# alibaba/TePDist

Measured on AMD Instinct MI355X. Metric: tokens/sec, higher is better.
Workload: dtype bf16; 1 GPU; model=gpt2-345m, global_batch=64, seq_len=1024, parallelism=auto-planned-graph:dp1tp1pp1mesh[]micro1

## Files before the change

### tepdist_amd/ops/build_ext.py

```python

from __future__ import annotations

import concurrent.futures as cf
import os
import subprocess
import sys
import sysconfig
from pathlib import Path

OPS_DIR = Path(__file__).resolve().parent
CSRC = OPS_DIR / "csrc"
OUT_SO = OPS_DIR / "_tepdist_hip.so"
BUILD = CSRC / "build"

HIPCC = os.environ.get("HIPCC", "/opt/rocm/bin/hipcc")
ARCH = os.environ.get("TEPDIST_GFX_ARCH", "gfx950")

SOURCES = [
    "gemm.hip",
    "gemm256.hip",
    "attention.hip",
    "decode_attention.hip",
    "transpose.hip",
    "layernorm.hip",
    "softmax.hip",
    "embedding.hip",
    "cross_entropy.hip",
    "dropout.hip",
    "elementwise.hip",
    "adamw.hip",
    "llama_ops.hip",
    "debug.hip",
    "bindings.cpp",
]


def _includes():
    import pybind11
    return [
        "-I", pybind11.get_include(),
        "-I", sysconfig.get_paths()["include"],
        "-I", str(CSRC),
    ]


def _needs_build() -> bool:
    if not OUT_SO.exists():
        return True
    so_mtime = OUT_SO.stat().st_mtime
    deps = [CSRC / s for s in SOURCES] + [CSRC / "common.h", CSRC / "kernels.h",
                                          Path(__file__)]
    return any(d.stat().st_mtime > so_mtime for d in deps)


RT_CSRC = OPS_DIR.parent / "runtime" / "csrc"
RT_SO = OPS_DIR.parent / "runtime" / "_tepdist_rt.so"
CXX = os.environ.get("CXX", "g++")


def build_rt(force: bool = False, verbose: bool = True) -> Path:
    src = RT_CSRC / "rt_core.cpp"
    if not force and RT_SO.exists() and \
            RT_SO.stat().st_mtime > src.stat().st_mtime:
        return RT_SO
    cmd = [CXX, "-O3", "-std=c++17", "-shared", "-fPIC",
           *_includes(), str(src), "-o", str(RT_SO)]
    if verbose:
        print("[build_ext]", " ".join(cmd), flush=True)
    r = subprocess.run(cmd, capture_output=True, text=True)
    if r.returncode != 0:
        raise RuntimeError(
            f"rt_core build failed:\n{r.stdout}\n{r.stderr}")
    return RT_SO


BLT_SO = OPS_DIR / "_tepdist_blt.so"


def build_blt(force: bool = False, verbose: bool = True) -> Path:
    src = CSRC / "blaslt.cpp"
    if not force and BLT_SO.exists() and \
            BLT_SO.stat().st_mtime > src.stat().st_mtime:
        return BLT_SO
    cmd = [HIPCC, "-O3", "-std=c++17", "-shared", "-fPIC",
           *_includes(), str(src), "-L", "/opt/rocm/lib", "-lhipblaslt",
           "-o", str(BLT_SO)]
    if verbose:
        print("[build_ext]", " ".join(cmd), flush=True)
    r = subprocess.run(cmd, capture_output=True, text=True)
    if r.returncode != 0:
        raise RuntimeError(f"blaslt build failed:\n{r.stdout}\n{r.stderr}")
    return BLT_SO


def build(force: bool = False, verbose: bool = True) -> Path:
    build_rt(force, verbose)
    build_blt(force, verbose)
    if not force and not _needs_build():
        return OUT_SO
    BUILD.mkdir(exist_ok=True)
    inc = _includes()
    base = [HIPCC, f"--offload-arch={ARCH}", "-O3", "-std=c++17", "-fPIC",
            "-Wno-unused-result"] + inc

    def compile_one(src: str) -> Path:
        obj = BUILD / (src.replace(".", "_") + ".o")
        lang = ["-x", "hip"] if src.endswith(".hip") else []
        cmd = base + lang + ["-c", str(CSRC / src), "-o", str(obj)]
        if verbose:
            print("[build_ext]", " ".join(cmd), flush=True)
        r = subprocess.run(cmd, capture_output=True, text=True)
        if r.returncode != 0:
            raise RuntimeError(
                f"hipcc failed for {src}:\n{r.stdout}\n{r.stderr}")
        return obj

    with cf.ThreadPoolExecutor(max_workers=min(8, len(SOURCES))) as ex:
        objs = list(ex.map(compile_one, SOURCES))

    link = [HIPCC, f"--offload-arch={ARCH}", "-shared", "-fPIC",
            *(str(o) for o in objs), "-o", str(OUT_SO)]
    if verbose:
        print("[build_ext]", " ".join(link), flush=True)
    r = subprocess.run(link, capture_output=True, text=True)
    if r.returncode != 0:
        raise RuntimeError(f"hipcc link failed:\n{r.stdout}\n{r.stderr}")
    return OUT_SO


if __name__ == "__main__":
    build(force="--force" in sys.argv)
    print(f"built {OUT_SO}")
```

### tepdist_amd/ops/csrc/attention.hip

```cpp

#include <algorithm>
#include <cstdlib>
#include <stdexcept>

#include "common.h"
#include "kernels.h"

namespace tepdist {

namespace {

constexpr int NT = 256;
constexpr int QB = 128;
constexpr int KB = 64;

template <int C>
DEV_INLINE int loff(int row, int col_e) {
  const int r1 = row >> 1;
  const int x = ((r1 & 1) << 2) | (r1 & 2) | ((r1 >> 2) & 1);
  return row * C + (col_e ^ ((x << 3) & (C - 1)));
}

DEV_INLINE float fast_exp(float x) {
  return __builtin_amdgcn_exp2f(x * 1.4426950408889634f);
}

#define BAR_LDS()                                        \
  do {                                                   \
    asm volatile("s_waitcnt lgkmcnt(0)" ::: "memory");   \
    __builtin_amdgcn_s_barrier();                        \
  } while (0)

DEV_INLINE float warp16_max(float v) {
#pragma unroll
  for (int d = 1; d < 16; d <<= 1) v = fmaxf(v, __shfl_xor(v, d, 64));
  return v;
}

DEV_INLINE float warp16_sum(float v) {
#pragma unroll
  for (int d = 1; d < 16; d <<= 1) v += __shfl_xor(v, d, 64);
  return v;
}


constexpr int NTF = 512;
constexpr int QBF = 512;

template <int D, int NQ = (D == 64 ? 4 : 2)>
__launch_bounds__(NTF) __global__
void flash_fwd_kernel(const bf16_t* __restrict__ Q,
                      const bf16_t* __restrict__ K,
                      const bf16_t* __restrict__ V, bf16_t* __restrict__ O,
                      float* __restrict__ LSE, int S, int H, float scale,
                      bool causal, int64_t q_bs, int64_t q_hs, int64_t q_rs,
                      int64_t o_bs, int64_t o_hs, int64_t o_rs) {
  constexpr int DK = D / 32;
  constexpr int DF = D / 16;
  const int bh = blockIdx.y;
  const int b = bh / H, h = bh % H;
  const int q0 = blockIdx.x * (128 * NQ);
  const int wave = threadIdx.x >> 6;
  const int lane = threadIdx.x & 63;
  const int g = lane >> 4;
  const int wq0 = q0 + wave * 16 * NQ;

  const bf16_t* qp = Q + (int64_t)b * q_bs + (int64_t)h * q_hs;
  const bf16_t* kp = K + (int64_t)b * q_bs + (int64_t)h * q_hs;
  const bf16_t* vp = V + (int64_t)b * q_bs + (int64_t)h * q_hs;
  bf16_t* op = O + (int64_t)b * o_bs + (int64_t)h * o_hs;

  __shared__ bf16_t smem[2 * (KB * D + D * KB)];
  const int BUFSZ = KB * D + D * KB;

  bf16x8 qf[NQ][DK];
#pragma unroll
  for (int nf = 0; nf < NQ; ++nf)
#pragma unroll
    for (int kk = 0; kk < DK; ++kk) {
      const int row = wq0 + nf * 16 + (lane & 15);
      bf16x8 v8 = {};
      if (row < S)
        v8 = *reinterpret_cast<const bf16x8*>(
            qp + (int64_t)row * q_rs + kk * 32 + 8 * g);
      qf[nf][kk] = v8;
    }

  f32x4 acc_o[DF][NQ] = {};
  float m_r[NQ], l_r[NQ];
#pragma unroll
  for (int i = 0; i < NQ; ++i) {
    m_r[i] = -3.0e38f;
    l_r[i] = 0.f;
  }

  constexpr int KUN = KB * D / 8 / NTF;
  constexpr int NSLAB = (KB / 8) * (D / 2);
  constexpr int SUN = (NSLAB + NTF - 1) / NTF;
  bf16x8 krg[KUN];
  uint32_t vrg[SUN][8];

  auto stage_load = [&](int kv0) {
#pragma unroll
    for (int u = 0; u < KUN; ++u) {
      const int idx = threadIdx.x + u * NTF;
      const int row = idx / (D / 8);
      const int c = (idx % (D / 8)) * 8;
      bf16x8 v8 = {};
      if (kv0 + row < S)
        v8 = *reinterpret_cast<const bf16x8*>(
            kp + (int64_t)(kv0 + row) * q_rs + c);
      krg[u] = v8;
    }
#pragma unroll
    for (int u = 0; u < SUN; ++u) {
      const int idx = threadIdx.x + u * NTF;
      if (idx >= NSLAB) break;
      const int f = 2 * (idx % (D / 2));
      const int kb = idx / (D / 2);
#pragma unroll
      for (int j = 0; j < 8; ++j) {
        const int kv = kv0 + kb * 8 + j;
        bf16x2 v2 = {};
        if (kv < S)
          v2 = *reinterpret_cast<const bf16x2*>(vp + (int64_t)kv * q_rs + f);
        vrg[u][j] = __builtin_bit_cast(uint32_t, v2);
      }
    }
  };
  auto stage_write = [&](int buf) {
    bf16_t* sK = smem + buf * BUFSZ;
    bf16_t* sVT = sK + KB * D;
#pragma unroll
    for (int u = 0; u < KUN; ++u) {
      const int idx = threadIdx.x + u * NTF;
      const int row = idx / (D / 8);
      const int c = (idx % (D / 8)) * 8;
      *reinterpret_cast<bf16x8*>(sK + loff<D>(row, c)) = krg[u];
    }
#pragma unroll
    for (int u = 0; u < SUN; ++u) {
      const int idx = threadIdx.x + u * NTF;
      if (idx >= NSLAB) break;
      const int f = 2 * (idx % (D / 2));
      const int kb = idx / (D / 2);
      uint32_t o0[4], o1[4];
#pragma unroll
      for (int d2 = 0; d2 < 4; ++d2) {
        o0[d2] = __builtin_amdgcn_perm(vrg[u][2 * d2 + 1], vrg[u][2 * d2],
                                       0x05040100u);
        o1[d2] = __builtin_amdgcn_perm(vrg[u][2 * d2 + 1], vrg[u][2 * d2],
                                       0x07060302u);
      }
      *reinterpret_cast<uint4*>(sVT + loff<KB>(f, kb * 8)) =
          make_uint4(o0[0], o0[1], o0[2], o0[3]);
      *reinterpret_cast<uint4*>(sVT + loff<KB>(f + 1, kb * 8)) =
          make_uint4(o1[0], o1[1], o1[2], o1[3]);
    }
  };

  const int kv_end = causal ? min(S, q0 + 128 * NQ) : S;
  stage_load(0);
  stage_write(0);
  __syncthreads();
  int t = 0;
  for (int kv0 = 0; kv0 < kv_end; kv0 += KB, ++t) {
    const bf16_t* sK = smem + (t & 1) * BUFSZ;
    const bf16_t* sVT = sK + KB * D;
    if (kv0 + KB < kv_end) stage_load(kv0 + KB);

    if (!causal || kv0 <= wq0 + 16 * NQ - 1) {
#pragma unroll
      for (int hp = 0; hp < NQ / 2; ++hp) {
        const int pq0 = wq0 + 32 * hp;
        if (causal && kv0 > pq0 + 31) continue;
        f32x4 st[4][2] = {};
        __builtin_amdgcn_s_setprio(1);
#pragma unroll
        for (int kk = 0; kk < DK; ++kk)
#pragma unroll
          for (int mi = 0; mi < 4; ++mi) {
            const bf16x8 kf = *reinterpret_cast<const bf16x8*>(
                sK + loff<D>((lane & 15) + 16 * mi, 8 * g + 32 * kk));
#pragma unroll
            for (int nf = 0; nf < 2; ++nf)
              st[mi][nf] = __builtin_amdgcn_mfma_f32_16x16x32_bf16(
                  kf, qf[2 * hp + nf][kk], st[mi][nf], 0, 0, 0);
          }
        __builtin_amdgcn_s_setprio(0);
        const bool inner = kv0 + KB <= pq0 && kv0 + KB <= S &&
                           pq0 + 32 <= S;
#pragma unroll
        for (int nf = 0; nf < 2; ++nf) {
          const int nfg = 2 * hp + nf;
          const int qg = pq0 + nf * 16 + (lane & 15);
          float tmax = -3.0e38f;
          if (inner) {
#pragma unroll
            for (int mi = 0; mi < 4; ++mi)
#pragma unroll
              for (int e = 0; e < 4; ++e) {
                const float sv = st[mi][nf][e] * scale;
                st[mi][nf][e] = sv;
                tmax = fmaxf(tmax, sv);
              }
          } else {
#pragma unroll
            for (int mi = 0; mi < 4; ++mi)
#pragma unroll
              for (int e = 0; e < 4; ++e) {
                const int kg = kv0 + mi * 16 + 4 * g + e;
                const bool masked = (causal && kg > qg) || kg >= S ||
                                    qg >= S;
                const float sv = masked ? -3.0e38f : st[mi][nf][e] * scale;
                st[mi][nf][e] = sv;
                tmax = fmaxf(tmax, sv);
              }
          }
          tmax = fmaxf(tmax, __shfl_xor(tmax, 16, 64));
          tmax = fmaxf(tmax, __shfl_xor(tmax, 32, 64));
          const float mn = fmaxf(m_r[nfg], tmax);
          const float alpha = fast_exp(m_r[nfg] - mn);
          m_r[nfg] = mn;
          float rs = 0.f;
#pragma unroll
          for (int mi = 0; mi < 4; ++mi)
#pragma unroll
            for (int e = 0; e < 4; ++e) {
              const float p = fast_exp(st[mi][nf][e] - mn);
              st[mi][nf][e] = p;
              rs += p;
            }
          rs += __shfl_xor(rs, 16, 64);
          rs += __shfl_xor(rs, 32, 64);
          l_r[nfg] = l_r[nfg] * alpha + rs;
#pragma unroll
          for (int df = 0; df < DF; ++df)
#pragma unroll
            for (int e = 0; e < 4; ++e) acc_o[df][nfg][e] *= alpha;
        }
        __builtin_amdgcn_s_setprio(1);
#pragma unroll
        for (int c = 0; c < KB / 32; ++c) {
          bf16x8 pb[2];
#pragma unroll
          for (int nf = 0; nf < 2; ++nf)
#pragma unroll
            for (int e = 0; e < 4; ++e) {
              pb[nf][e] = f2bf(st[2 * c][nf][e]);
              pb[nf][e + 4] = f2bf(st[2 * c + 1][nf][e]);
            }
#pragma unroll
          for (int df = 0; df < DF; ++df) {
            const bf16x4 v0 = *reinterpret_cast<const bf16x4*>(
                sVT + loff<KB>(16 * df + (lane & 15), 32 * c + 4 * g));
            const bf16x4 v1 = *reinterpret_cast<const bf16x4*>(
                sVT + loff<KB>(16 * df + (lane & 15), 32 * c + 16 + 4 * g));
            bf16x8 vfr;
#pragma unroll
            for (int e = 0; e < 4; ++e) {
              vfr[e] = v0[e];
              vfr[e + 4] = v1[e];
            }
#pragma unroll
            for (int nf = 0; nf < 2; ++nf)
              acc_o[df][2 * hp + nf] = __builtin_amdgcn_mfma_f32_16x16x32_bf16(
                  vfr, pb[nf], acc_o[df][2 * hp + nf], 0, 0, 0);
          }
        }
        __builtin_amdgcn_s_setprio(0);
      }
    }
    if (kv0 + KB < kv_end) stage_write((t + 1) & 1);
    BAR_LDS();
  }

#pragma unroll
  for (int nf = 0; nf < NQ; ++nf) {
    const int qg = wq0 + nf * 16 + (lane & 15);
    if (qg >= S) continue;
    const float lv = l_r[nf];
    const float inv = (lv > 0.f) ? 1.0f / lv : 0.f;
    if (g == 0)
      LSE[(int64_t)bh * S + qg] =
          (lv > 0.f) ? m_r[nf] + __logf(lv) : -3.0e38f;
#pragma unroll
    for (int df = 0; df < DF; ++df)
#pragma unroll
      for (int e = 0; e < 4; ++e)
        op[(int64_t)qg * o_rs + 16 * df + 4 * g + e] =
            f2bf(acc_o[df][nf][e] * inv);
  }
}

}

void attention_fwd_bf16(const void* q, const void* k, const void* v, void* o,
                        float* lse, int B, int H, int S, int D, float scale,
                        bool causal, int64_t q_bs, int64_t q_hs, int64_t q_rs,
                        int64_t o_bs, int64_t o_hs, int64_t o_rs,
                        hipStream_t stream) {
  dim3 block(NTF);
#define FWD_D(DD)                                                        \
  do {                                                                   \
    dim3 grid((S + (DD == 64 ? QBF : 256) - 1) / (DD == 64 ? QBF : 256), \
              B * H);                                                    \
    hipLaunchKernelGGL(flash_fwd_kernel<DD>, grid, block, 0, stream,     \
                       static_cast<const bf16_t*>(q),                    \
                       static_cast<const bf16_t*>(k),                    \
                       static_cast<const bf16_t*>(v),                    \
                       static_cast<bf16_t*>(o), lse, S, H, scale,        \
                       causal, q_bs, q_hs, q_rs, o_bs, o_hs, o_rs);      \
  } while (0)
  if (D == 64) FWD_D(64);
  else if (D == 128) FWD_D(128);
  else throw std::runtime_error("flash fwd: head dim must be 64 or 128");
#undef FWD_D
}

namespace {


template <int D>
__launch_bounds__(NT) __global__
void flash_bwd_delta_kernel(const bf16_t* __restrict__ dO,
                            const bf16_t* __restrict__ O,
                            float* __restrict__ delta, int64_t rows) {
  const int lane = threadIdx.x & 63;
  const int wid = threadIdx.x >> 6;
  const int64_t nw = (int64_t)gridDim.x * (NT / WAVE);
  for (int64_t r = (int64_t)blockIdx.x * (NT / WAVE) + wid; r < rows;
       r += nw) {
    float s = 0.f;
    for (int c = lane * 8; c < D; c += WAVE * 8) {
      const bf16x8 a = *reinterpret_cast<const bf16x8*>(dO + r * D + c);
      const bf16x8 b = *reinterpret_cast<const bf16x8*>(O + r * D + c);
#pragma unroll
      for (int e = 0; e < 8; ++e) s += bf2f(a[e]) * bf2f(b[e]);
    }
    s = wave_allreduce_sum(s);
    if (lane == 0) delta[r] = s;
  }
}

template <int T, int D>
DEV_INLINE void stage_nat_t(const bf16_t* __restrict__ src, int row0, int S,
                            int64_t rs, bf16_t* nat, bf16_t* tr) {
  constexpr int UN = T * D / 8 / NT;
#pragma unroll
  for (int u = 0; u < UN; ++u) {
    const int idx = threadIdx.x + u * NT;
    const int row = idx / (D / 8);
    const int c = (idx % (D / 8)) * 8;
    bf16x8 v8 = {};
    if (row0 + row < S)
      v8 = *reinterpret_cast<const bf16x8*>(
          src + (int64_t)(row0 + row) * rs + c);
    *reinterpret_cast<bf16x8*>(nat + loff<D>(row, c)) = v8;
  }
  constexpr int NSLAB = (T / 8) * (D / 2);
#pragma unroll
  for (int u = 0; u < (NSLAB + NT - 1) / NT; ++u) {
    const int idx = threadIdx.x + u * NT;
    if (idx < NSLAB) {
      const int f = 2 * (idx % (D / 2));
      const int kb = idx / (D / 2);
      uint32_t r[8];
#pragma unroll
      for (int j = 0; j < 8; ++j) {
        const int row = row0 + kb * 8 + j;
        bf16x2 v2 = {};
        if (row < S)
          v2 = *reinterpret_cast<const bf16x2*>(src + (int64_t)row * rs + f);
        r[j] = __builtin_bit_cast(uint32_t, v2);
      }
      uint32_t o0[4], o1[4];
#pragma unroll
      for (int d2 = 0; d2 < 4; ++d2) {
        o0[d2] = __builtin_amdgcn_perm(r[2 * d2 + 1], r[2 * d2], 0x05040100u);
        o1[d2] = __builtin_amdgcn_perm(r[2 * d2 + 1], r[2 * d2], 0x07060302u);
      }
      *reinterpret_cast<uint4*>(tr + loff<T>(f, kb * 8)) =
          make_uint4(o0[0], o0[1], o0[2], o0[3]);
      *reinterpret_cast<uint4*>(tr + loff<T>(f + 1, kb * 8)) =
          make_uint4(o1[0], o1[1], o1[2], o1[3]);
    }
  }
}

constexpr int NTA = 512;

template <int D, int PROBE = 0, int KBA = (D == 64 ? 256 : 128)>
__launch_bounds__(NTA) __global__
void flash_bwd_kv_kernel(const bf16_t* __restrict__ Q,
                         const bf16_t* __restrict__ K,
                         const bf16_t* __restrict__ V,
                         const bf16_t* __restrict__ dO,
                         const float* __restrict__ LSE,
                         const float* __restrict__ DELTA,
                         bf16_t* __restrict__ dK, bf16_t* __restrict__ dV,
                         int S, int H, float scale, bool causal,
                         int64_t q_bs, int64_t q_hs, int64_t q_rs,
                         int64_t o_bs, int64_t o_hs, int64_t o_rs) {
  constexpr int DK = D / 32;
  constexpr int DF = D / 16;
  constexpr int QT = 64;
  constexpr int NSL = KBA / 128;
  const int bh = blockIdx.y;
  const int b = bh / H, h = bh % H;
  const int kv0 = blockIdx.x * KBA;
  const int wave = threadIdx.x >> 6;
  const int lane = threadIdx.x & 63;
  const int g = lane >> 4;

  const int64_t qoff = (int64_t)b * q_bs + (int64_t)h * q_hs;
  const int64_t ooff = (int64_t)b * o_bs + (int64_t)h * o_hs;
  const bf16_t* qp = Q + qoff;
  const bf16_t* kp = K + qoff;
  const bf16_t* vp = V + qoff;
  const bf16_t* dop = dO + ooff;

  __shared__ bf16_t smem[KBA * D * 2 + QT * D * 2 + D * QT * 2];
  bf16_t* sKb = smem;
  bf16_t* sVb = sKb + KBA * D;
  bf16_t* sQ = sVb + KBA * D;
  bf16_t* sQT = sQ + QT * D;
  bf16_t* sdO = sQT + D * QT;
  bf16_t* sdOT = sdO + QT * D;
  __shared__ float sLSE[QT], sDELTA[QT];

  {
    constexpr int UN = KBA * D / 8 / NTA;
#pragma unroll
    for (int u = 0; u < UN; ++u) {
      const int idx = threadIdx.x + u * NTA;
      const int row = idx / (D / 8);
      const int c = (idx % (D / 8)) * 8;
      bf16x8 kv8 = {}, vv8 = {};
      if (kv0 + row < S) {
        kv8 = *reinterpret_cast<const bf16x8*>(
            kp + (int64_t)(kv0 + row) * q_rs + c);
        vv8 = *reinterpret_cast<const bf16x8*>(
            vp + (int64_t)(kv0 + row) * q_rs + c);
      }
      *reinterpret_cast<bf16x8*>(sKb + loff<D>(row, c)) = kv8;
      *reinterpret_cast<bf16x8*>(sVb + loff<D>(row, c)) = vv8;
    }
  }
  __syncthreads();

  f32x4 acc_dkT[NSL][DF] = {};
  f32x4 acc_dvT[NSL][DF] = {};

  constexpr int QUN = QT * D / 8 / NTA;
  constexpr int TSLAB = (QT / 8) * (D / 2);
  constexpr int TUN = (TSLAB + NTA - 1) / NTA;
  bf16x8 qn[QUN], don[QUN];
  uint32_t qt[TUN][8], dot_[TUN][8];
  float lse2[QT / NTA + 1], dl2[QT / NTA + 1];

  auto tile_load = [&](int q0) {
#pragma unroll
    for (int u = 0; u < QUN; ++u) {
      const int idx = threadIdx.x + u * NTA;
      const int row = idx / (D / 8);
      const int c = (idx % (D / 8)) * 8;
      bf16x8 a = {}, b2 = {};
      if (q0 + row < S) {
        a = *reinterpret_cast<const bf16x8*>(
            qp + (int64_t)(q0 + row) * q_rs + c);
        b2 = *reinterpret_cast<const bf16x8*>(
            dop + (int64_t)(q0 + row) * o_rs + c);
      }
      qn[u] = a;
      don[u] = b2;
    }
#pragma unroll
    for (int u = 0; u < TUN; ++u) {
      const int idx = threadIdx.x + u * NTA;
      if (idx >= TSLAB) break;
      const int f = 2 * (idx % (D / 2));
      const int kb = idx / (D / 2);
#pragma unroll
      for (int j = 0; j < 8; ++j) {
        const int row = q0 + kb * 8 + j;
        bf16x2 a = {}, b2 = {};
        if (row < S) {
          a = *reinterpret_cast<const bf16x2*>(
              qp + (int64_t)row * q_rs + f);
          b2 = *reinterpret_cast<const bf16x2*>(
              dop + (int64_t)row * o_rs + f);
        }
        qt[u][j] = __builtin_bit_cast(uint32_t, a);
        dot_[u][j] = __builtin_bit_cast(uint32_t, b2);
      }
    }
    for (int i = threadIdx.x, s2 = 0; i < QT; i += NTA, ++s2) {
      const int qg = q0 + i;
      lse2[s2] = (qg < S) ? LSE[(int64_t)bh * S + qg] : -3.0e38f;
      dl2[s2] = (qg < S) ? DELTA[(int64_t)bh * S + qg] : 0.f;
    }
  };
  auto tile_write = [&]() {
#pragma unroll
    for (int u = 0; u < QUN; ++u) {
      const int idx = threadIdx.x + u * NTA;
      const int row = idx / (D / 8);
      const int c = (idx % (D / 8)) * 8;
      *reinterpret_cast<bf16x8*>(sQ + loff<D>(row, c)) = qn[u];
      *reinterpret_cast<bf16x8*>(sdO + loff<D>(row, c)) = don[u];
    }
#pragma unroll
    for (int u = 0; u < TUN; ++u) {
      const int idx = threadIdx.x + u * NTA;
      if (idx >= TSLAB) break;
      const int f = 2 * (idx % (D / 2));
      const int kb = idx / (D / 2);
      uint32_t o0[4], o1[4];
#pragma unroll
      for (int d2 = 0; d2 < 4; ++d2) {
        o0[d2] = __builtin_amdgcn_perm(qt[u][2 * d2 + 1], qt[u][2 * d2],
                                       0x05040100u);
        o1[d2] = __builtin_amdgcn_perm(qt[u][2 * d2 + 1], qt[u][2 * d2],
                                       0x07060302u);
      }
      *reinterpret_cast<uint4*>(sQT + loff<QT>(f, kb * 8)) =
          make_uint4(o0[0], o0[1], o0[2], o0[3]);
      *reinterpret_cast<uint4*>(sQT + loff<QT>(f + 1, kb * 8)) =
          make_uint4(o1[0], o1[1], o1[2], o1[3]);
#pragma unroll
      for (int d2 = 0; d2 < 4; ++d2) {
        o0[d2] = __builtin_amdgcn_perm(dot_[u][2 * d2 + 1], dot_[u][2 * d2],
                                       0x05040100u);
        o1[d2] = __builtin_amdgcn_perm(dot_[u][2 * d2 + 1], dot_[u][2 * d2],
                                       0x07060302u);
      }
      *reinterpret_cast<uint4*>(sdOT + loff<QT>(f, kb * 8)) =
          make_uint4(o0[0], o0[1], o0[2], o0[3]);
      *reinterpret_cast<uint4*>(sdOT + loff<QT>(f + 1, kb * 8)) =
          make_uint4(o1[0], o1[1], o1[2], o1[3]);
    }
    for (int i = threadIdx.x, s2 = 0; i < QT; i += NTA, ++s2) {
      sLSE[i] = lse2[s2];
      sDELTA[i] = dl2[s2];
    }
  };

  const int q_start = causal ? (kv0 / QT) * QT : 0;
  tile_load(q_start);
  tile_write();
  __syncthreads();
  for (int q0 = q_start; q0 < S; q0 += QT) {
    if (q0 + QT < S) tile_load(q0 + QT);

#pragma unroll
    for (int sl = 0; sl < NSL; ++sl) {
      f32x4 st[4] = {};
      f32x4 dpt[4] = {};
#pragma unroll
      for (int kk = 0; kk < DK; ++kk) {
        const bf16x8 kfr = *reinterpret_cast<const bf16x8*>(
            sKb + loff<D>(sl * 128 + wave * 16 + (lane & 15),
                          8 * g + 32 * kk));
        const bf16x8 vfr = *reinterpret_cast<const bf16x8*>(
            sVb + loff<D>(sl * 128 + wave * 16 + (lane & 15),
                          8 * g + 32 * kk));
#pragma unroll
        for (int mi = 0; mi < 4; ++mi) {
          const bf16x8 qa = *reinterpret_cast<const bf16x8*>(
              sQ + loff<D>(16 * mi + (lane & 15), 8 * g + 32 * kk));
          st[mi] = __builtin_amdgcn_mfma_f32_16x16x32_bf16(qa, kfr,
                                                           st[mi], 0, 0, 0);
          const bf16x8 da = *reinterpret_cast<const bf16x8*>(
              sdO + loff<D>(16 * mi + (lane & 15), 8 * g + 32 * kk));
          dpt[mi] = __builtin_amdgcn_mfma_f32_16x16x32_bf16(
              da, vfr, dpt[mi], 0, 0, 0);
        }
      }

      const int kvb = kv0 + sl * 128;
      const int kvg = kvb + wave * 16 + (lane & 15);
      const bool winner = (!causal || kvb + wave * 16 + 15 < q0) &&
                          q0 + QT <= S && kvb + 128 <= S;
      if (winner) {
        f32x4 lsev[4], dlv[4];
#pragma unroll
        for (int mi = 0; mi < 4; ++mi) {
          lsev[mi] = *reinterpret_cast<const f32x4*>(sLSE + 16 * mi + 4 * g);
          dlv[mi] = *reinterpret_cast<const f32x4*>(sDELTA + 16 * mi + 4 * g);
        }
#pragma unroll
        for (int mi = 0; mi < 4; ++mi)
#pragma unroll
          for (int e = 0; e < 4; ++e) {
            const float pt = fast_exp(st[mi][e] * scale - lsev[mi][e]);
            st[mi][e] = pt;
            dpt[mi][e] = pt * (dpt[mi][e] - dlv[mi][e]) * scale;
          }
      } else {
#pragma unroll
        for (int mi = 0; mi < 4; ++mi)
#pragma unroll
          for (int e = 0; e < 4; ++e) {
            const int qrow = 16 * mi + 4 * g + e;
            const int qg = q0 + qrow;
            const float lse = sLSE[qrow];
            const float dl = sDELTA[qrow];
            const bool valid = qg < S && kvg < S && (!causal || kvg <= qg) &&
                               lse > -1.0e38f;
            const float arg = valid ? st[mi][e] * scale - lse : -3.0e38f;
            const float pt = fast_exp(arg);
            st[mi][e] = pt;
            dpt[mi][e] = pt * (dpt[mi][e] - dl) * scale;
          }
      }

      __builtin_amdgcn_s_setprio(1);
#pragma unroll
      for (int c = 0; c < QT / 32; ++c) {
        bf16x8 pb, db;
#pragma unroll
        for (int e = 0; e < 4; ++e) {
          pb[e] = f2bf(st[2 * c][e]);
          pb[e + 4] = f2bf(st[2 * c + 1][e]);
          db[e] = f2bf(dpt[2 * c][e]);
          db[e + 4] = f2bf(dpt[2 * c + 1][e]);
        }
#pragma unroll
        for (int df = 0; df < DF; ++df) {
          const int fr = PROBE ? 0 : (lane & 15);
          const bf16x4 a0 = *reinterpret_cast<const bf16x4*>(
              sdOT + loff<QT>(16 * df + fr, 32 * c + 4 * g));
          const bf16x4 a1 = *reinterpret_cast<const bf16x4*>(
              sdOT + loff<QT>(16 * df + fr, 32 * c + 16 + 4 * g));
          const bf16x4 q0f = *reinterpret_cast<const bf16x4*>(
              sQT + loff<QT>(16 * df + fr, 32 * c + 4 * g));
          const bf16x4 q1f = *reinterpret_cast<const bf16x4*>(
              sQT + loff<QT>(16 * df + fr, 32 * c + 16 + 4 * g));
          bf16x8 afr, qfr;
#pragma unroll
          for (int e = 0; e < 4; ++e) {
            afr[e] = a0[e];
            afr[e + 4] = a1[e];
            qfr[e] = q0f[e];
            qfr[e + 4] = q1f[e];
          }
          acc_dvT[sl][df] = __builtin_amdgcn_mfma_f32_16x16x32_bf16(
              afr, pb, acc_dvT[sl][df], 0, 0, 0);
          acc_dkT[sl][df] = __builtin_amdgcn_mfma_f32_16x16x32_bf16(
              qfr, db, acc_dkT[sl][df], 0, 0, 0);
        }
      }
      __builtin_amdgcn_s_setprio(0);
    }
    BAR_LDS();
    if (q0 + QT < S) {
      tile_write();
      BAR_LDS();
    }
  }

#pragma unroll
  for (int sl = 0; sl < NSL; ++sl) {
    const int kvg = kv0 + sl * 128 + wave * 16 + (lane & 15);
    if (kvg < S) {
#pragma unroll
      for (int df = 0; df < DF; ++df) {
        bf16x4 kv4, vv4;
#pragma unroll
        for (int e = 0; e < 4; ++e) {
          kv4[e] = f2bf(acc_dkT[sl][df][e]);
          vv4[e] = f2bf(acc_dvT[sl][df][e]);
        }
        const int64_t off = qoff + (int64_t)kvg * q_rs + 16 * df + 4 * g;
        *reinterpret_cast<bf16x4*>(dK + off) = kv4;
        *reinterpret_cast<bf16x4*>(dV + off) = vv4;
      }
    }
  }
}

constexpr int NTB = 512;
constexpr int QBB = 256;

template <int D, int NQ = (D == 64 ? 4 : 2)>
__launch_bounds__(NTB) __global__
void flash_bwd_dq_kernel(const bf16_t* __restrict__ Q,
                         const bf16_t* __restrict__ K,
                         const bf16_t* __restrict__ V,
                         const bf16_t* __restrict__ dO,
                         const float* __restrict__ LSE,
                         const float* __restrict__ DELTA,
                         bf16_t* __restrict__ dQ, int S, int H, float scale,
                         bool causal, int64_t q_bs, int64_t q_hs,
                         int64_t q_rs, int64_t o_bs, int64_t o_hs,
                         int64_t o_rs) {
  constexpr int DK = D / 32;
  constexpr int DF = D / 16;
  const int bh = blockIdx.y;
  const int b = bh / H, h = bh % H;
  const int q0 = blockIdx.x * (128 * NQ);
  const int wave = threadIdx.x >> 6;
  const int lane = threadIdx.x & 63;
  const int g = lane >> 4;
  const int wq0 = q0 + wave * 16 * NQ;

  const int64_t qoff = (int64_t)b * q_bs + (int64_t)h * q_hs;
  const int64_t ooff = (int64_t)b * o_bs + (int64_t)h * o_hs;
  const bf16_t* qp = Q + qoff;
  const bf16_t* kp = K + qoff;
  const bf16_t* vp = V + qoff;
  const bf16_t* dop = dO + ooff;
  bf16_t* dqp = dQ + qoff;

  __shared__ bf16_t smem[KB * D * 2 + D * KB];
  bf16_t* sK = smem;
  bf16_t* sV = smem + KB * D;
  bf16_t* sKT = sV + KB * D;

  bf16x8 qf[NQ][DK], dof[NQ][DK];
  float lse_r[NQ], dl_r[NQ];
#pragma unroll
  for (int nf = 0; nf < NQ; ++nf) {
    const int row = wq0 + nf * 16 + (lane & 15);
    lse_r[nf] = (row < S) ? LSE[(int64_t)bh * S + row] : -3.0e38f;
    dl_r[nf] = (row < S) ? DELTA[(int64_t)bh * S + row] : 0.f;
#pragma unroll
    for (int kk = 0; kk < DK; ++kk) {
      bf16x8 a = {}, b8 = {};
      if (row < S) {
        a = *reinterpret_cast<const bf16x8*>(
            qp + (int64_t)row * q_rs + kk * 32 + 8 * g);
        b8 = *reinterpret_cast<const bf16x8*>(
            dop + (int64_t)row * o_rs + kk * 32 + 8 * g);
      }
      qf[nf][kk] = a;
      dof[nf][kk] = b8;
    }
  }

  f32x4 acc_dq[DF][NQ] = {};

  constexpr int KUN = KB * D / 8 / NTB;
  constexpr int NSLAB = (KB / 8) * (D / 2);
  constexpr int SUN = (NSLAB + NTB - 1) / NTB;
  bf16x8 krg[KUN], vrg[KUN];
  uint32_t ktr[SUN][8];

  auto stage_load = [&](int kv0) {
#pragma unroll
    for (int u = 0; u < KUN; ++u) {
      const int idx = threadIdx.x + u * NTB;
      const int row = idx / (D / 8);
      const int c = (idx % (D / 8)) * 8;
      bf16x8 kv8 = {}, vv8 = {};
      if (kv0 + row < S) {
        kv8 = *reinterpret_cast<const bf16x8*>(
            kp + (int64_t)(kv0 + row) * q_rs + c);
        vv8 = *reinterpret_cast<const bf16x8*>(
            vp + (int64_t)(kv0 + row) * q_rs + c);
      }
      krg[u] = kv8;
      vrg[u] = vv8;
    }
#pragma unroll
    for (int u = 0; u < SUN; ++u) {
      const int idx = threadIdx.x + u * NTB;
      if (idx >= NSLAB) break;
      const int f = 2 * (idx % (D / 2));
      const int kb = idx / (D / 2);
#pragma unroll
      for (int j = 0; j < 8; ++j) {
        const int kv = kv0 + kb * 8 + j;
        bf16x2 v2 = {};
        if (kv < S)
          v2 = *reinterpret_cast<const bf16x2*>(kp + (int64_t)kv * q_rs + f);
        ktr[u][j] = __builtin_bit_cast(uint32_t, v2);
      }
    }
  };
  auto stage_write = [&]() {
#pragma unroll
    for (int u = 0; u < KUN; ++u) {
      const int idx = threadIdx.x + u * NTB;
      const int row = idx / (D / 8);
      const int c = (idx % (D / 8)) * 8;
      *reinterpret_cast<bf16x8*>(sK + loff<D>(row, c)) = krg[u];
      *reinterpret_cast<bf16x8*>(sV + loff<D>(row, c)) = vrg[u];
    }
#pragma unroll
    for (int u = 0; u < SUN; ++u) {
      const int idx = threadIdx.x + u * NTB;
      if (idx >= NSLAB) break;
      const int f = 2 * (idx % (D / 2));
      const int kb = idx / (D / 2);
      uint32_t o0[4], o1[4];
#pragma unroll
      for (int d2 = 0; d2 < 4; ++d2) {
        o0[d2] = __builtin_amdgcn_perm(ktr[u][2 * d2 + 1], ktr[u][2 * d2],
                                       0x05040100u);
        o1[d2] = __builtin_amdgcn_perm(ktr[u][2 * d2 + 1], ktr[u][2 * d2],
                                       0x07060302u);
      }
      *reinterpret_cast<uint4*>(sKT + loff<KB>(f, kb * 8)) =
          make_uint4(o0[0], o0[1], o0[2], o0[3]);
      *reinterpret_cast<uint4*>(sKT + loff<KB>(f + 1, kb * 8)) =
          make_uint4(o1[0], o1[1], o1[2], o1[3]);
    }
  };

  const int kv_end = causal ? min(S, q0 + 128 * NQ) : S;
  stage_load(0);
  stage_write();
  __syncthreads();
  for (int kv0 = 0; kv0 < kv_end; kv0 += KB) {
    if (kv0 + KB < kv_end) stage_load(kv0 + KB);

    if (!causal || kv0 <= wq0 + 16 * NQ - 1) {
#pragma unroll
     for (int hp = 0; hp < NQ / 2; ++hp) {
      const int pq0 = wq0 + 32 * hp;
      if (causal && kv0 > pq0 + 31) continue;
      const bool inner = kv0 + KB <= pq0 && kv0 + KB <= S && pq0 + 32 <= S;
      bf16x4 dsb[4][2];
#pragma unroll
      for (int mi = 0; mi < 4; ++mi) {
        f32x4 st[2] = {};
        f32x4 dpt[2] = {};
        __builtin_amdgcn_s_setprio(1);
#pragma unroll
        for (int kk = 0; kk < DK; ++kk) {
          const bf16x8 ka = *reinterpret_cast<const bf16x8*>(
              sK + loff<D>((lane & 15) + 16 * mi, 8 * g + 32 * kk));
          const bf16x8 va = *reinterpret_cast<const bf16x8*>(
              sV + loff<D>((lane & 15) + 16 * mi, 8 * g + 32 * kk));
#pragma unroll
          for (int nf = 0; nf < 2; ++nf) {
            st[nf] = __builtin_amdgcn_mfma_f32_16x16x32_bf16(
                ka, qf[2 * hp + nf][kk], st[nf], 0, 0, 0);
            dpt[nf] = __builtin_amdgcn_mfma_f32_16x16x32_bf16(
                va, dof[2 * hp + nf][kk], dpt[nf], 0, 0, 0);
          }
        }
        __builtin_amdgcn_s_setprio(0);
#pragma unroll
        for (int nf = 0; nf < 2; ++nf) {
          const int nfg = 2 * hp + nf;
          const int qg = pq0 + nf * 16 + (lane & 15);
          if (inner) {
#pragma unroll
            for (int e = 0; e < 4; ++e) {
              const float pt = fast_exp(st[nf][e] * scale - lse_r[nfg]);
              dsb[mi][nf][e] =
                  f2bf(pt * (dpt[nf][e] - dl_r[nfg]) * scale);
            }
          } else {
#pragma unroll
            for (int e = 0; e < 4; ++e) {
              const int kg = kv0 + 16 * mi + 4 * g + e;
              const bool valid = qg < S && kg < S &&
                                 (!causal || kg <= qg) &&
                                 lse_r[nfg] > -1.0e38f;
              const float arg = valid ? st[nf][e] * scale - lse_r[nfg]
                                      : -3.0e38f;
              const float pt = fast_exp(arg);
              dsb[mi][nf][e] =
                  f2bf(pt * (dpt[nf][e] - dl_r[nfg]) * scale);
            }
          }
        }
      }
      __builtin_amdgcn_s_setprio(1);
#pragma unroll
      for (int c = 0; c < KB / 32; ++c) {
        bf16x8 db[2];
#pragma unroll
        for (int nf = 0; nf < 2; ++nf)
#pragma unroll
          for (int e = 0; e < 4; ++e) {
            db[nf][e] = dsb[2 * c][nf][e];
            db[nf][e + 4] = dsb[2 * c + 1][nf][e];
          }
#pragma unroll
        for (int df = 0; df < DF; ++df) {
          const bf16x4 k0 = *reinterpret_cast<const bf16x4*>(
              sKT + loff<KB>(16 * df + (lane & 15), 32 * c + 4 * g));
          const bf16x4 k1 = *reinterpret_cast<const bf16x4*>(
              sKT + loff<KB>(16 * df + (lane & 15), 32 * c + 16 + 4 * g));
          bf16x8 kfr;
#pragma unroll
          for (int e = 0; e < 4; ++e) {
            kfr[e] = k0[e];
            kfr[e + 4] = k1[e];
          }
#pragma unroll
          for (int nf = 0; nf < 2; ++nf)
            acc_dq[df][2 * hp + nf] = __builtin_amdgcn_mfma_f32_16x16x32_bf16(
                kfr, db[nf], acc_dq[df][2 * hp + nf], 0, 0, 0);
        }
      }
      __builtin_amdgcn_s_setprio(0);
     }
    }
    BAR_LDS();
    if (kv0 + KB < kv_end) {
      stage_write();
      BAR_LDS();
    }
  }

#pragma unroll
  for (int nf = 0; nf < NQ; ++nf) {
    const int qg = wq0 + nf * 16 + (lane & 15);
    if (qg >= S) continue;
#pragma unroll
    for (int df = 0; df < DF; ++df) {
      bf16x4 v4;
#pragma unroll
      for (int e = 0; e < 4; ++e) v4[e] = f2bf(acc_dq[df][nf][e]);
      *reinterpret_cast<bf16x4*>(
          dqp + (int64_t)qg * q_rs + 16 * df + 4 * g) = v4;
    }
  }
}


template <int D>
__global__ void flash_bwd_delta_strided_kernel(
    const bf16_t* __restrict__ dO, const bf16_t* __restrict__ O,
    float* __restrict__ delta, int H, int S, int64_t o_bs, int64_t o_hs,
    int64_t o_rs) {
  constexpr int LPR = D / 8;
  constexpr int RPW = WAVE / LPR;
  const int lane = threadIdx.x & 63;
  const int wid = threadIdx.x >> 6;
  const int sub = lane / LPR;
  const int c = (lane % LPR) * 8;
  const int64_t nr = (int64_t)gridDim.x * (NT / WAVE) * RPW;
  const int bh = blockIdx.y;
  const int b = bh / H, h = bh % H;
  const int64_t off = (int64_t)b * o_bs + (int64_t)h * o_hs;
  for (int64_t r0 = ((int64_t)blockIdx.x * (NT / WAVE) + wid) * RPW;
       r0 < S; r0 += nr) {
    const int64_t r = r0 + sub;
    float s = 0.f;
    if (r < S) {
      const bf16x8 a =
          *reinterpret_cast<const bf16x8*>(dO + off + r * o_rs + c);
      const bf16x8 bb =
          *reinterpret_cast<const bf16x8*>(O + off + r * o_rs + c);
#pragma unroll
      for (int e = 0; e < 8; ++e) s += bf2f(a[e]) * bf2f(bb[e]);
    }
#pragma unroll
    for (int d2 = 1; d2 < LPR; d2 <<= 1) s += __shfl_xor(s, d2, 64);
    if (r < S && (lane % LPR) == 0) delta[(int64_t)bh * S + r] = s;
  }
}

}



void attention_bwd_bf16(const void* q, const void* k, const void* v,
                        const void* o, const void* dout, const float* lse,
                        float* delta, void* dq, void* dk, void* dv,
                        int B, int H, int S, int D, float scale, bool causal,
                        int64_t q_bs, int64_t q_hs, int64_t q_rs,
                        int64_t o_bs, int64_t o_hs, int64_t o_rs,
                        hipStream_t stream) {
  dim3 block(NT);
#define BWD_D(DD)                                                            \
  do {                                                                       \
    dim3 dgrid((S / 4 + (NT / WAVE) - 1) / (NT / WAVE) > 256                 \
                   ? 256 : (S + 3) / 4, B * H);                              \
    hipLaunchKernelGGL(flash_bwd_delta_strided_kernel<DD>, dgrid, block, 0,  \
                       stream, static_cast<const bf16_t*>(dout),             \
                       static_cast<const bf16_t*>(o), delta, H, S, o_bs,     \
                       o_hs, o_rs);                                          \
    dim3 kgrid((S + (DD == 64 ? 255 : 127)) / (DD == 64 ? 256 : 128),       \
               B * H);                                                       \
    static const bool kv_probe = std::getenv("TEPDIST_FLASH_PROBE");         \
    if (kv_probe)                                                            \
      hipLaunchKernelGGL((flash_bwd_kv_kernel<DD, 1>), kgrid, dim3(512), 0,  \
                         stream, static_cast<const bf16_t*>(q),              \
                         static_cast<const bf16_t*>(k),                      \
                         static_cast<const bf16_t*>(v),                      \
                         static_cast<const bf16_t*>(dout), lse, delta,       \
                         static_cast<bf16_t*>(dk), static_cast<bf16_t*>(dv), \
                         S, H, scale, causal, q_bs, q_hs, q_rs, o_bs, o_hs,  \
                         o_rs);                                              \
    else                                                                     \
    hipLaunchKernelGGL(flash_bwd_kv_kernel<DD>, kgrid, dim3(512), 0, stream, \
                       static_cast<const bf16_t*>(q),                        \
                       static_cast<const bf16_t*>(k),                        \
                       static_cast<const bf16_t*>(v),                        \
                       static_cast<const bf16_t*>(dout), lse, delta,         \
                       static_cast<bf16_t*>(dk), static_cast<bf16_t*>(dv),   \
                       S, H, scale, causal, q_bs, q_hs, q_rs, o_bs, o_hs,    \
                       o_rs);                                                \
    dim3 qgrid((S + (DD == 64 ? 511 : 255)) / (DD == 64 ? 512 : 256),       \
               B * H);                                                       \
    hipLaunchKernelGGL(flash_bwd_dq_kernel<DD>, qgrid, dim3(NTB), 0, stream, \
                       static_cast<const bf16_t*>(q),                        \
                       static_cast<const bf16_t*>(k),                        \
                       static_cast<const bf16_t*>(v),                        \
                       static_cast<const bf16_t*>(dout), lse, delta,         \
                       static_cast<bf16_t*>(dq), S, H, scale, causal, q_bs,  \
                       q_hs, q_rs, o_bs, o_hs, o_rs);                        \
  } while (0)
  if (D == 64) BWD_D(64);
  else if (D == 128) BWD_D(128);
  else throw std::runtime_error("flash bwd: head dim must be 64 or 128");
#undef BWD_D
}
}
```

### tepdist_amd/ops/csrc/bindings.cpp

```cpp

#include <pybind11/pybind11.h>

#include <hip/hip_runtime.h>

#include "common.h"
#include "kernels.h"

namespace py = pybind11;
using namespace tepdist;

namespace {

hipStream_t S(uintptr_t s) { return reinterpret_cast<hipStream_t>(s); }

void check_launch() { HIP_CHECK(hipGetLastError()); }

}

PYBIND11_MODULE(_tepdist_hip, m) {
  m.doc() = "TePDist-AMD gfx950 kernel library";

  m.def("gemm", [](uintptr_t A, uintptr_t B, uintptr_t C, uintptr_t Cpre,
                   uintptr_t bias, int M, int N, int K, int lda, int ldb,
                   int ldc, int64_t sa, int64_t sb, int64_t sc, int batch,
                   bool a_kc, bool b_kc, int epi, int split_k,
                   uintptr_t stream) {
    gemm_bf16(reinterpret_cast<void*>(A), reinterpret_cast<void*>(B),
              reinterpret_cast<void*>(C), reinterpret_cast<void*>(Cpre),
              reinterpret_cast<void*>(bias), M, N, K, lda, ldb, ldc, sa, sb,
              sc, batch, a_kc, b_kc, epi, split_k, S(stream));
    check_launch();
  });

  m.def("splitk_reduce", [](uintptr_t parts, uintptr_t out, int nparts,
                            int64_t mn, uintptr_t stream) {
    splitk_reduce(reinterpret_cast<const float*>(parts),
                  reinterpret_cast<void*>(out), nparts, mn, S(stream));
    check_launch();
  });

  m.def("transpose", [](uintptr_t in, uintptr_t out, int R, int C,
                        int64_t si, int64_t so, int batch,
                        uintptr_t stream) {
    transpose_bf16(reinterpret_cast<void*>(in), reinterpret_cast<void*>(out),
                   R, C, si, so, batch, S(stream));
    check_launch();
  });

  m.def("layernorm_fwd", [](uintptr_t x, uintptr_t g, uintptr_t b, uintptr_t y,
                            uintptr_t mean, uintptr_t rstd, int rows, int cols,
                            float eps, uintptr_t stream, uintptr_t res,
                            uintptr_t sum_out) {
    layernorm_fwd_bf16(reinterpret_cast<void*>(x), reinterpret_cast<void*>(g),
                       reinterpret_cast<void*>(b), reinterpret_cast<void*>(y),
                       reinterpret_cast<float*>(mean),
                       reinterpret_cast<float*>(rstd), rows, cols, eps,
                       S(stream), reinterpret_cast<void*>(res),
                       reinterpret_cast<void*>(sum_out));
    check_launch();
  }, pybind11::arg("x"), pybind11::arg("g"), pybind11::arg("b"),
     pybind11::arg("y"), pybind11::arg("mean"), pybind11::arg("rstd"),
     pybind11::arg("rows"), pybind11::arg("cols"), pybind11::arg("eps"),
     pybind11::arg("stream"), pybind11::arg("res") = 0,
     pybind11::arg("sum_out") = 0);

  m.def("layernorm_bwd", [](uintptr_t dy, uintptr_t x, uintptr_t g,
                            uintptr_t mean, uintptr_t rstd, uintptr_t dx,
                            uintptr_t dg_part, uintptr_t db_part,
                            uintptr_t dgamma, uintptr_t dbeta, int rows,
                            int cols, int part_rows, uintptr_t stream,
                            uintptr_t dsum) {
    layernorm_bwd_bf16(reinterpret_cast<void*>(dy), reinterpret_cast<void*>(x),
                       reinterpret_cast<void*>(g),
                       reinterpret_cast<float*>(mean),
                       reinterpret_cast<float*>(rstd),
                       reinterpret_cast<void*>(dx),
                       reinterpret_cast<float*>(dg_part),
                       reinterpret_cast<float*>(db_part), rows, cols,
                       part_rows, S(stream), reinterpret_cast<void*>(dsum));
    check_launch();
    layernorm_bwd_reduce(reinterpret_cast<float*>(dg_part),
                         reinterpret_cast<float*>(db_part),
                         reinterpret_cast<void*>(dgamma),
                         reinterpret_cast<void*>(dbeta), part_rows, cols,
                         S(stream));
    check_launch();
  }, pybind11::arg("dy"), pybind11::arg("x"), pybind11::arg("g"),
     pybind11::arg("mean"), pybind11::arg("rstd"), pybind11::arg("dx"),
     pybind11::arg("dg_part"), pybind11::arg("db_part"),
     pybind11::arg("dgamma"), pybind11::arg("dbeta"), pybind11::arg("rows"),
     pybind11::arg("cols"), pybind11::arg("part_rows"),
     pybind11::arg("stream"), pybind11::arg("dsum") = 0);

  m.def("softmax_fwd", [](uintptr_t x, uintptr_t p, int64_t rows, int cols,
                          int sq, float scale, bool causal, uintptr_t stream) {
    softmax_fwd_bf16(reinterpret_cast<void*>(x), reinterpret_cast<void*>(p),
                     rows, cols, sq, scale, causal, S(stream));
    check_launch();
  });

  m.def("softmax_bwd", [](uintptr_t dp, uintptr_t p, uintptr_t ds,
                          int64_t rows, int cols, float scale,
                          uintptr_t stream) {
    softmax_bwd_bf16(reinterpret_cast<void*>(dp), reinterpret_cast<void*>(p),
                     reinterpret_cast<void*>(ds), rows, cols, scale,
                     S(stream));
    check_launch();
  });

  m.def("attention_fwd", [](uintptr_t q, uintptr_t k, uintptr_t v,
                            uintptr_t o, uintptr_t lse, int B, int H,
                            int seq, int D, float scale, bool causal,
                            int64_t q_bs, int64_t q_hs, int64_t q_rs,
                            int64_t o_bs, int64_t o_hs, int64_t o_rs,
                            uintptr_t stream) {
    attention_fwd_bf16(reinterpret_cast<void*>(q), reinterpret_cast<void*>(k),
                       reinterpret_cast<void*>(v), reinterpret_cast<void*>(o),
                       reinterpret_cast<float*>(lse), B, H, seq, D, scale,
                       causal, q_bs, q_hs, q_rs, o_bs, o_hs, o_rs, S(stream));
    check_launch();
  });

  m.def("attention_bwd", [](uintptr_t q, uintptr_t k, uintptr_t v,
                            uintptr_t o, uintptr_t dout, uintptr_t lse,
                            uintptr_t delta, uintptr_t dq, uintptr_t dk,
                            uintptr_t dv, int B, int H, int seq, int D,
                            float scale, bool causal, int64_t q_bs,
                            int64_t q_hs, int64_t q_rs, int64_t o_bs,
                            int64_t o_hs, int64_t o_rs, uintptr_t stream) {
    attention_bwd_bf16(
        reinterpret_cast<void*>(q), reinterpret_cast<void*>(k),
        reinterpret_cast<void*>(v), reinterpret_cast<void*>(o),
        reinterpret_cast<void*>(dout), reinterpret_cast<float*>(lse),
        reinterpret_cast<float*>(delta), reinterpret_cast<void*>(dq),
        reinterpret_cast<void*>(dk), reinterpret_cast<void*>(dv), B, H, seq,
        D, scale, causal, q_bs, q_hs, q_rs, o_bs, o_hs, o_rs, S(stream));
    check_launch();
  });

  m.def("decode_attention", [](uintptr_t q, uintptr_t k_new, uintptr_t v_new,
                               uintptr_t k_cache, uintptr_t v_cache,
                               uintptr_t pos, int pos_stride, uintptr_t out,
                               uintptr_t ws, int B, int H, int S_max, int D,
                               float scale, int splits, int64_t q_bs,
                               int64_t q_hs, int64_t n_bs, int64_t n_hs,
                               int64_t c_bs, int64_t c_hs, int64_t c_rs,
                               uintptr_t stream) {
    decode_attention_bf16(
        reinterpret_cast<void*>(q), reinterpret_cast<void*>(k_new),
        reinterpret_cast<void*>(v_new), reinterpret_cast<void*>(k_cache),
        reinterpret_cast<void*>(v_cache),
        reinterpret_cast<const int64_t*>(pos), pos_stride,
        reinterpret_cast<void*>(out), reinterpret_cast<float*>(ws), B, H,
        S_max, D, scale, splits, q_bs, q_hs, n_bs, n_hs, c_bs, c_hs, c_rs,
        S(stream));
    check_launch();
  });

  m.def("embedding_fwd",[](uintptr_t ids, uintptr_t table, uintptr_t out,
                            int64_t n_ids, int dim, uintptr_t stream) {
    embedding_fwd_bf16(reinterpret_cast<const int64_t*>(ids),
                       reinterpret_cast<void*>(table),
                       reinterpret_cast<void*>(out), n_ids, dim, S(stream));
    check_launch();
  });

  m.def("embedding_bwd", [](uintptr_t dy, uintptr_t ids, uintptr_t grad_f32,
                            uintptr_t grad_bf16, int64_t n_ids, int vocab,
                            int dim, uintptr_t stream) {
    embedding_bwd_bf16(reinterpret_cast<void*>(dy),
                       reinterpret_cast<const int64_t*>(ids),
                       reinterpret_cast<float*>(grad_f32),
                       reinterpret_cast<void*>(grad_bf16), n_ids, vocab, dim,
                       S(stream));
    check_launch();
  });

  m.def("cross_entropy_fwd", [](uintptr_t logits, uintptr_t targets,
                                uintptr_t nll, uintptr_t lse, int64_t rows,
                                int cols, int ignore, uintptr_t stream) {
    cross_entropy_fwd_bf16(reinterpret_cast<void*>(logits),
                           reinterpret_cast<const int64_t*>(targets),
                           reinterpret_cast<float*>(nll),
                           reinterpret_cast<float*>(lse), rows, cols, ignore,
                           S(stream));
    check_launch();
  });

  m.def("cross_entropy_bwd", [](uintptr_t logits, uintptr_t targets,
                                uintptr_t lse, uintptr_t dscale,
                                uintptr_t dlogits, int64_t rows, int cols,
                                int ignore, uintptr_t stream) {
    cross_entropy_bwd_bf16(reinterpret_cast<void*>(logits),
                           reinterpret_cast<const int64_t*>(targets),
                           reinterpret_cast<const float*>(lse),
                           reinterpret_cast<const float*>(dscale),
                           reinterpret_cast<void*>(dlogits), rows, cols,
                           ignore, S(stream));
    check_launch();
  });

  m.def("dropout_fwd", [](uintptr_t x, uintptr_t y, uintptr_t mask, int64_t n,
                          float p, uint64_t seed, uint64_t offset,
                          uintptr_t stream) {
    dropout_fwd_bf16(reinterpret_cast<void*>(x), reinterpret_cast<void*>(y),
                     reinterpret_cast<uint8_t*>(mask), n, p, seed, offset,
                     S(stream));
    check_launch();
  });

  m.def("dropout_bwd", [](uintptr_t dy, uintptr_t mask, uintptr_t dx,
                          int64_t n, float p, uintptr_t stream) {
    dropout_bwd_bf16(reinterpret_cast<void*>(dy),
                     reinterpret_cast<const uint8_t*>(mask),
                     reinterpret_cast<void*>(dx), n, p, S(stream));
    check_launch();
  });

  m.def("gelu_fwd", [](uintptr_t x, uintptr_t y, int64_t n, uintptr_t stream) {
    gelu_fwd_bf16(reinterpret_cast<void*>(x), reinterpret_cast<void*>(y), n,
                  S(stream));
    check_launch();
  });

  m.def("cast_ws", [](uintptr_t ws, uintptr_t db, int cols,
                      uintptr_t stream) {
    cast_ws_f32_bf16(reinterpret_cast<const float*>(ws),
                     reinterpret_cast<void*>(db), cols, S(stream));
    check_launch();
  });
  m.def("transpose_dy", [](uintptr_t dy, uintptr_t pre, uintptr_t dgt,
                           uintptr_t dgn, uintptr_t bias_ws, int R, int C,
                           uintptr_t stream) {
    transpose_dy_bf16(reinterpret_cast<void*>(dy),
                      reinterpret_cast<void*>(pre),
                      reinterpret_cast<void*>(dgt),
                      reinterpret_cast<void*>(dgn),
                      reinterpret_cast<float*>(bias_ws), R, C, S(stream));
    check_launch();
  });
  m.def("rmsnorm_fwd", [](uintptr_t x, uintptr_t g, uintptr_t y,
                          uintptr_t rstd, int64_t rows, int cols, float eps,
                          uintptr_t stream) {
    rmsnorm_fwd_bf16(reinterpret_cast<void*>(x), reinterpret_cast<void*>(g),
                     reinterpret_cast<void*>(y),
                     reinterpret_cast<float*>(rstd), rows, cols, eps,
                     S(stream));
    check_launch();
  });
  m.def("rmsnorm_bwd", [](uintptr_t dy, uintptr_t x, uintptr_t g,
                          uintptr_t rstd, uintptr_t dx, uintptr_t dg,
                          uintptr_t dg_part, int part_rows, int64_t rows,
                          int cols, uintptr_t stream) {
    rmsnorm_bwd_bf16(reinterpret_cast<void*>(dy), reinterpret_cast<void*>(x),
                     reinterpret_cast<void*>(g),
                     reinterpret_cast<const float*>(rstd),
                     reinterpret_cast<void*>(dx), reinterpret_cast<void*>(dg),
                     reinterpret_cast<float*>(dg_part), part_rows, rows,
                     cols, S(stream));
    check_launch();
  });
  m.def("rope", [](uintptr_t x, uintptr_t y, int64_t tokens, int heads,
                   int D, int seq_len, float theta, bool backward,
                   uintptr_t stream) {
    rope_bf16(reinterpret_cast<void*>(x), reinterpret_cast<void*>(y), tokens,
              heads, D, seq_len, theta, backward, S(stream));
    check_launch();
  });
  m.def("swiglu_fwd", [](uintptr_t a, uintptr_t b, uintptr_t y, int64_t n,
                         uintptr_t stream) {
    swiglu_fwd_bf16(reinterpret_cast<void*>(a), reinterpret_cast<void*>(b),
                    reinterpret_cast<void*>(y), n, S(stream));
    check_launch();
  });
  m.def("swiglu_bwd", [](uintptr_t dy, uintptr_t a, uintptr_t b,
                         uintptr_t da, uintptr_t db, int64_t n,
                         uintptr_t stream) {
    swiglu_bwd_bf16(reinterpret_cast<void*>(dy), reinterpret_cast<void*>(a),
                    reinterpret_cast<void*>(b), reinterpret_cast<void*>(da),
                    reinterpret_cast<void*>(db), n, S(stream));
    check_launch();
  });
  m.def("gelu_bwd", [](uintptr_t dy, uintptr_t x, uintptr_t dx, int64_t n,
                       uintptr_t stream) {
    gelu_bwd_bf16(reinterpret_cast<void*>(dy), reinterpret_cast<void*>(x),
                  reinterpret_cast<void*>(dx), n, S(stream));
    check_launch();
  });

  m.def("bias_sum", [](uintptr_t dy, uintptr_t db, uintptr_t ws, int64_t rows,
                       int cols, uintptr_t stream) {
    bias_sum_bf16(reinterpret_cast<void*>(dy), reinterpret_cast<void*>(db),
                  reinterpret_cast<float*>(ws), rows, cols, S(stream));
    check_launch();
  });

  m.def("adamw", [](uintptr_t param, uintptr_t master, uintptr_t grad_bf16,
                    uintptr_t grad_f32, uintptr_t m_, uintptr_t v_, int64_t n,
                    float lr, float b1, float b2, float eps, float wd,
                    float bc1, float bc2, uintptr_t stream) {
    adamw_bf16(reinterpret_cast<void*>(param),
               reinterpret_cast<float*>(master),
               reinterpret_cast<void*>(grad_bf16),
               reinterpret_cast<const float*>(grad_f32),
               reinterpret_cast<float*>(m_), reinterpret_cast<float*>(v_), n,
               lr, b1, b2, eps, wd, bc1, bc2, S(stream));
    check_launch();
  });

  m.def("tr16_probe", [](uintptr_t a, uintptr_t b, uintptr_t stream) {
    tr16_probe(reinterpret_cast<float*>(a), reinterpret_cast<float*>(b),
               S(stream));
  });

  m.def("adamw_mt", [](uintptr_t tabs, uintptr_t numel, uintptr_t wds,
                       uintptr_t ptypes, uintptr_t chunks, int nchunks,
                       int nt, float lr, float b1, float b2, float eps,
                       float bc1, float bc2, uintptr_t hyper,
                       uintptr_t stream) {
    adamw_mt_bf16(reinterpret_cast<const int64_t*>(tabs),
                  reinterpret_cast<const int64_t*>(numel),
                  reinterpret_cast<const float*>(wds),
                  reinterpret_cast<const unsigned char*>(ptypes),
                  reinterpret_cast<const int*>(chunks), nchunks, nt, lr, b1,
                  b2, eps, bc1, bc2,
                  reinterpret_cast<const float*>(hyper), S(stream));
    check_launch();
  });

  m.def("device_sync", []() { HIP_CHECK(hipDeviceSynchronize()); });
}
```

### tepdist_amd/ops/csrc/debug.hip

```cpp

#include "common.h"
#include "kernels.h"

namespace tepdist {

namespace {

typedef __attribute__((address_space(3))) bf16x4* lds_tr_ptr;

__global__ void tr16_probe_kernel(float* out_pattern, float* out_uniform) {
  __shared__ bf16_t lds[512];
  for (int i = threadIdx.x; i < 512; i += blockDim.x)
    lds[i] = f2bf((float)i);
  __syncthreads();
  if (threadIdx.x < 64) {
    const int lane = threadIdx.x;
    const bf16_t* p =
        &lds[0] + (lane & 15) + (lane >> 4) * 64;
    bf16x4 v = __builtin_amdgcn_ds_read_tr16_b64_v4bf16((lds_tr_ptr)p);
#pragma unroll
    for (int j = 0; j < 4; ++j) out_pattern[lane * 4 + j] = bf2f(v[j]);
    bf16x4 u = __builtin_amdgcn_ds_read_tr16_b64_v4bf16((lds_tr_ptr)&lds[0]);
#pragma unroll
    for (int j = 0; j < 4; ++j) out_uniform[lane * 4 + j] = bf2f(u[j]);
  }
}

}

void tr16_probe(float* out_pattern, float* out_uniform, hipStream_t stream) {
  hipLaunchKernelGGL(tr16_probe_kernel, dim3(1), dim3(64), 0, stream,
                     out_pattern, out_uniform);
  HIP_CHECK(hipGetLastError());
}

}
```

### tepdist_amd/ops/csrc/kernels.h

```cpp
#pragma once

#include <hip/hip_runtime.h>
#include <hip/hip_bf16.h>
#include <cstdint>

namespace tepdist {

using bf16 = __hip_bfloat16;

void gemm_bf16(const void* A, const void* B, void* C, void* c_pre,
               const void* bias, int M, int N, int K, int lda, int ldb,
               int ldc, int64_t stride_a, int64_t stride_b, int64_t stride_c,
               int batch, bool a_kc, bool b_kc, int epi, int split_k,
               hipStream_t stream);
bool gemm256_supported(int M, int N, int K, int lda, int ldb, bool a_kc,
                       bool b_kc, int epi, int split_k);
void gemm256_bf16(const void* A, const void* B, void* C, void* c_pre,
                  const void* bias, int M, int N, int K, int lda, int ldb,
                  int ldc, int64_t stride_a, int64_t stride_b,
                  int64_t stride_c, int batch, int epi, int split_k,
                  hipStream_t stream);
void splitk_reduce(const float* parts, void* out, int nparts, int64_t mn,
                   hipStream_t stream);

void transpose_bf16(const void* in, void* out, int R, int C,
                    int64_t stride_in, int64_t stride_out, int batch,
                    hipStream_t stream);
void cast_ws_f32_bf16(const float* ws, void* db_out, int cols,
                      hipStream_t stream);
void transpose_dy_bf16(const void* dy, const void* pre, void* dy_t,
                       void* dy_nat, float* bias_ws, int R, int C,
                       hipStream_t stream);

void layernorm_fwd_bf16(const void* x, const void* gamma, const void* beta,
                        void* y, float* mean, float* rstd, int rows, int cols,
                        float eps, hipStream_t stream,
                        const void* res = nullptr, void* sum_out = nullptr);
void layernorm_bwd_bf16(const void* dy, const void* x, const void* gamma,
                        const float* mean, const float* rstd, void* dx,
                        float* dgamma_part, float* dbeta_part, int rows,
                        int cols, int part_rows, hipStream_t stream,
                        const void* dsum = nullptr);
void layernorm_bwd_reduce(const float* dgamma_part, const float* dbeta_part,
                          void* dgamma, void* dbeta, int part_rows, int cols,
                          hipStream_t stream);

void softmax_fwd_bf16(const void* x, void* p, int64_t rows, int cols, int sq,
                      float scale, bool causal, hipStream_t stream);
void softmax_bwd_bf16(const void* dp, const void* p, void* ds, int64_t rows,
                      int cols, float scale, hipStream_t stream);

void attention_fwd_bf16(const void* q, const void* k, const void* v, void* o,
                        float* lse, int B, int H, int S, int D, float scale,
                        bool causal, int64_t q_bs, int64_t q_hs, int64_t q_rs,
                        int64_t o_bs, int64_t o_hs, int64_t o_rs,
                        hipStream_t stream);
void attention_bwd_bf16(const void* q, const void* k, const void* v,
                        const void* o, const void* dout, const float* lse,
                        float* delta, void* dq, void* dk, void* dv,
                        int B, int H, int S, int D, float scale, bool causal,
                        int64_t q_bs, int64_t q_hs, int64_t q_rs,
                        int64_t o_bs, int64_t o_hs, int64_t o_rs,
                        hipStream_t stream);

void decode_attention_bf16(const void* q, const void* k_new,
                           const void* v_new, void* k_cache, void* v_cache,
                           const int64_t* pos, int pos_stride, void* out,
                           float* ws, int B, int H, int S_max, int D,
                           float scale, int splits, int64_t q_bs,
                           int64_t q_hs, int64_t n_bs, int64_t n_hs,
                           int64_t c_bs, int64_t c_hs, int64_t c_rs,
                           hipStream_t stream);

void embedding_fwd_bf16(const int64_t* ids, const void* table, void* out,
                        int64_t n_ids, int dim, hipStream_t stream);
void embedding_bwd_bf16(const void* dy, const int64_t* ids, float* grad_f32,
                        void* grad_bf16, int64_t n_ids, int vocab, int dim,
                        hipStream_t stream);

void cross_entropy_fwd_bf16(const void* logits, const int64_t* targets,
                            float* nll, float* lse, int64_t rows, int cols,
                            int ignore_index, hipStream_t stream);
void cross_entropy_bwd_bf16(const void* logits, const int64_t* targets,
                            const float* lse, const float* dscale,
                            void* dlogits, int64_t rows, int cols,
                            int ignore_index, hipStream_t stream);

void dropout_fwd_bf16(const void* x, void* y, uint8_t* mask, int64_t n,
                      float p, uint64_t seed, uint64_t offset,
                      hipStream_t stream);
void dropout_bwd_bf16(const void* dy, const uint8_t* mask, void* dx, int64_t n,
                      float p, hipStream_t stream);

void gelu_fwd_bf16(const void* x, void* y, int64_t n, hipStream_t stream);
void gelu_bwd_bf16(const void* dy, const void* x, void* dx, int64_t n,
                   hipStream_t stream);
void bias_sum_bf16(const void* dy, void* db, float* ws_zeroed, int64_t rows,
                   int cols, hipStream_t stream);

void adamw_bf16(void* param, float* master, const void* grad_bf16,
                const float* grad_f32, float* exp_avg, float* exp_avg_sq,
                int64_t n, float lr, float beta1, float beta2, float eps,
                float weight_decay, float bc1, float bc2, hipStream_t stream);

void adamw_mt_bf16(const int64_t* tabs, const int64_t* numel,
                   const float* wds, const unsigned char* ptypes,
                   const int* chunks, int nchunks, int nt,
                   float lr, float beta1, float beta2, float eps, float bc1,
                   float bc2, const float* hyper, hipStream_t stream);

void tr16_probe(float* out_pattern, float* out_uniform, hipStream_t stream);

void rmsnorm_fwd_bf16(const void* x, const void* g, void* y, float* rstd,
                      int64_t rows, int cols, float eps, hipStream_t stream);
void rmsnorm_bwd_bf16(const void* dy, const void* x, const void* g,
                      const float* rstd, void* dx, void* dgamma,
                      float* dg_part, int part_rows, int64_t rows, int cols,
                      hipStream_t stream);
void rope_bf16(const void* x, void* y, int64_t tokens, int heads, int D,
               int seq_len, float theta, bool backward, hipStream_t stream);
void swiglu_fwd_bf16(const void* a, const void* b, void* y, int64_t n,
                     hipStream_t stream);
void swiglu_bwd_bf16(const void* dy, const void* a, const void* b, void* da,
                     void* db, int64_t n, hipStream_t stream);

}
```

Baseline: 295,900 tokens/s.

## Use ds_read_tr16 transposed LDS reads in flash attention, drop explicit transposes

Result: faster. 309,100 tokens/s, median of 6 (+4.5%).

```diff
diff --git a/tepdist_amd/ops/build_ext.py b/tepdist_amd/ops/build_ext.py
--- a/tepdist_amd/ops/build_ext.py
+++ b/tepdist_amd/ops/build_ext.py
@@ -49,6 +49,7 @@
         return True
     so_mtime = OUT_SO.stat().st_mtime
     deps = [CSRC / s for s in SOURCES] + [CSRC / "common.h", CSRC / "kernels.h",
+                                          CSRC / "lds_frag.h",
                                           Path(__file__)]
     return any(d.stat().st_mtime > so_mtime for d in deps)
 
diff --git a/tepdist_amd/ops/csrc/attention.hip b/tepdist_amd/ops/csrc/attention.hip
--- a/tepdist_amd/ops/csrc/attention.hip
+++ b/tepdist_amd/ops/csrc/attention.hip
@@ -1,10 +1,10 @@
 
 #include <algorithm>
-#include <cstdlib>
 #include <stdexcept>
 
 #include "common.h"
 #include "kernels.h"
+#include "lds_frag.h"
 
 namespace tepdist {
 
@@ -14,15 +14,9 @@
 constexpr int QB = 128;
 constexpr int KB = 64;
 
-template <int C>
-DEV_INLINE int loff(int row, int col_e) {
-  const int r1 = row >> 1;
-  const int x = ((r1 & 1) << 2) | (r1 & 2) | ((r1 >> 2) & 1);
-  return row * C + (col_e ^ ((x << 3) & (C - 1)));
-}
-
+constexpr float kLog2e = 1.4426950408889634f;
 DEV_INLINE float fast_exp(float x) {
-  return __builtin_amdgcn_exp2f(x * 1.4426950408889634f);
+  return __builtin_amdgcn_exp2f(x * kLog2e);
 }
 
 #define BAR_LDS()                                        \
@@ -46,6 +40,11 @@
 
 constexpr int NTF = 512;
 constexpr int QBF = 512;
+
+template <int NQ>
+DEV_INLINE int pair_row0(int q0, int wave, int hp) {
+  return NQ == 4 ? q0 + 32 * (hp ? 15 - wave : wave) : q0 + 32 * wave;
+}
 
 template <int D, int NQ = (D == 64 ? 4 : 2)>
 __launch_bounds__(NTF) __global__
@@ -60,25 +59,25 @@
   const int bh = blockIdx.y;
   const int b = bh / H, h = bh % H;
   const int q0 = blockIdx.x * (128 * NQ);
-  const int wave = threadIdx.x >> 6;
+  const int wave = __builtin_amdgcn_readfirstlane(threadIdx.x >> 6);
   const int lane = threadIdx.x & 63;
   const int g = lane >> 4;
-  const int wq0 = q0 + wave * 16 * NQ;
 
   const bf16_t* qp = Q + (int64_t)b * q_bs + (int64_t)h * q_hs;
   const bf16_t* kp = K + (int64_t)b * q_bs + (int64_t)h * q_hs;
   const bf16_t* vp = V + (int64_t)b * q_bs + (int64_t)h * q_hs;
   bf16_t* op = O + (int64_t)b * o_bs + (int64_t)h * o_hs;
 
-  __shared__ bf16_t smem[2 * (KB * D + D * KB)];
-  const int BUFSZ = KB * D + D * KB;
+  __shared__ __attribute__((aligned(16))) bf16_t smem[2 * 2 * KB * D];
+  const int BUFSZ = 2 * KB * D;
 
   bf16x8 qf[NQ][DK];
 #pragma unroll
   for (int nf = 0; nf < NQ; ++nf)
 #pragma unroll
     for (int kk = 0; kk < DK; ++kk) {
-      const int row = wq0 + nf * 16 + (lane & 15);
+      const int row = pair_row0<NQ>(q0, wave, nf >> 1) + (nf & 1) * 16 +
+                      (lane & 15);
       bf16x8 v8 = {};
       if (row < S)
         v8 = *reinterpret_cast<const bf16x8*>(
@@ -86,6 +85,7 @@
       qf[nf][kk] = v8;
     }
 
+  const float sl2 = scale * kLog2e;
   f32x4 acc_o[DF][NQ] = {};
   float m_r[NQ], l_r[NQ];
 #pragma unroll
@@ -95,10 +95,7 @@
   }
 
   constexpr int KUN = KB * D / 8 / NTF;
-  constexpr int NSLAB = (KB / 8) * (D / 2);
-  constexpr int SUN = (NSLAB + NTF - 1) / NTF;
-  bf16x8 krg[KUN];
-  uint32_t vrg[SUN][8];
+  bf16x8 krg[KUN], vrg[KUN];
 
   auto stage_load = [&](int kv0) {
 #pragma unroll
@@ -106,56 +103,27 @@
       const int idx = threadIdx.x + u * NTF;
       const int row = idx / (D / 8);
       const int c = (idx % (D / 8)) * 8;
-      bf16x8 v8 = {};
-      if (kv0 + row < S)
+      bf16x8 k8 = {}, v8 = {};
+      if (kv0 + row < S) {
+        k8 = *reinterpret_cast<const bf16x8*>(
+            kp + (int64_t)(kv0 + row) * q_rs + c);
         v8 = *reinterpret_cast<const bf16x8*>(
-            kp + (int64_t)(kv0 + row) * q_rs + c);
-      krg[u] = v8;
-    }
-#pragma unroll
-    for (int u = 0; u < SUN; ++u) {
-      const int idx = threadIdx.x + u * NTF;
-      if (idx >= NSLAB) break;
-      const int f = 2 * (idx % (D / 2));
-      const int kb = idx / (D / 2);
-#pragma unroll
-      for (int j = 0; j < 8; ++j) {
-        const int kv = kv0 + kb * 8 + j;
-        bf16x2 v2 = {};
-        if (kv < S)
-          v2 = *reinterpret_cast<const bf16x2*>(vp + (int64_t)kv * q_rs + f);
-        vrg[u][j] = __builtin_bit_cast(uint32_t, v2);
-      }
+            vp + (int64_t)(kv0 + row) * q_rs + c);
+      }
+      krg[u] = k8;
+      vrg[u] = v8;
     }
   };
   auto stage_write = [&](int buf) {
     bf16_t* sK = smem + buf * BUFSZ;
-    bf16_t* sVT = sK + KB * D;
+    bf16_t* sV = sK + KB * D;
 #pragma unroll
     for (int u = 0; u < KUN; ++u) {
       const int idx = threadIdx.x + u * NTF;
       const int row = idx / (D / 8);
       const int c = (idx % (D / 8)) * 8;
       *reinterpret_cast<bf16x8*>(sK + loff<D>(row, c)) = krg[u];
-    }
-#pragma unroll
-    for (int u = 0; u < SUN; ++u) {
-      const int idx = threadIdx.x + u * NTF;
-      if (idx >= NSLAB) break;
-      const int f = 2 * (idx % (D / 2));
-      const int kb = idx / (D / 2);
-      uint32_t o0[4], o1[4];
-#pragma unroll
-      for (int d2 = 0; d2 < 4; ++d2) {
-        o0[d2] = __builtin_amdgcn_perm(vrg[u][2 * d2 + 1], vrg[u][2 * d2],
-                                       0x05040100u);
-        o1[d2] = __builtin_amdgcn_perm(vrg[u][2 * d2 + 1], vrg[u][2 * d2],
-                                       0x07060302u);
-      }
-      *reinterpret_cast<uint4*>(sVT + loff<KB>(f, kb * 8)) =
-          make_uint4(o0[0], o0[1], o0[2], o0[3]);
-      *reinterpret_cast<uint4*>(sVT + loff<KB>(f + 1, kb * 8)) =
-          make_uint4(o1[0], o1[1], o1[2], o1[3]);
+      *reinterpret_cast<bf16x8*>(sV + loff<D>(row, c)) = vrg[u];
     }
   };
 
@@ -166,13 +134,13 @@
   int t = 0;
   for (int kv0 = 0; kv0 < kv_end; kv0 += KB, ++t) {
     const bf16_t* sK = smem + (t & 1) * BUFSZ;
-    const bf16_t* sVT = sK + KB * D;
+    const bf16_t* sV = sK + KB * D;
     if (kv0 + KB < kv_end) stage_load(kv0 + KB);
 
-    if (!causal || kv0 <= wq0 + 16 * NQ - 1) {
+    if (!causal || kv0 <= pair_row0<NQ>(q0, wave, NQ / 2 - 1) + 31) {
 #pragma unroll
       for (int hp = 0; hp < NQ / 2; ++hp) {
-        const int pq0 = wq0 + 32 * hp;
+        const int pq0 = pair_row0<NQ>(q0, wave, hp);
         if (causal && kv0 > pq0 + 31) continue;
         f32x4 st[4][2] = {};
         __builtin_amdgcn_s_setprio(1);
@@ -199,11 +167,8 @@
 #pragma unroll
             for (int mi = 0; mi < 4; ++mi)
 #pragma unroll
-              for (int e = 0; e < 4; ++e) {
-                const float sv = st[mi][nf][e] * scale;
-                st[mi][nf][e] = sv;
-                tmax = fmaxf(tmax, sv);
-              }
+              for (int e = 0; e < 4; ++e)
+                tmax = fmaxf(tmax, st[mi][nf][e]);
           } else {
 #pragma unroll
             for (int mi = 0; mi < 4; ++mi)
@@ -212,22 +177,24 @@
                 const int kg = kv0 + mi * 16 + 4 * g + e;
                 const bool masked = (causal && kg > qg) || kg >= S ||
                                     qg >= S;
-                const float sv = masked ? -3.0e38f : st[mi][nf][e] * scale;
+                const float sv = masked ? -3.0e38f : st[mi][nf][e];
                 st[mi][nf][e] = sv;
                 tmax = fmaxf(tmax, sv);
               }
           }
           tmax = fmaxf(tmax, __shfl_xor(tmax, 16, 64));
           tmax = fmaxf(tmax, __shfl_xor(tmax, 32, 64));
-          const float mn = fmaxf(m_r[nfg], tmax);
+          const float mn = fmaxf(m_r[nfg], tmax * scale);
           const float alpha = fast_exp(m_r[nfg] - mn);
           m_r[nfg] = mn;
+          const float nm2 = -mn * kLog2e;
           float rs = 0.f;
 #pragma unroll
           for (int mi = 0; mi < 4; ++mi)
 #pragma unroll
             for (int e = 0; e < 4; ++e) {
-              const float p = fast_exp(st[mi][nf][e] - mn);
+              const float p = __builtin_amdgcn_exp2f(
+                  __builtin_fmaf(st[mi][nf][e], sl2, nm2));
               st[mi][nf][e] = p;
               rs += p;
             }
@@ -252,16 +219,7 @@
             }
 #pragma unroll
           for (int df = 0; df < DF; ++df) {
-            const bf16x4 v0 = *reinterpret_cast<const bf16x4*>(
-                sVT + loff<KB>(16 * df + (lane & 15), 32 * c + 4 * g));
-            const bf16x4 v1 = *reinterpret_cast<const bf16x4*>(
-                sVT + loff<KB>(16 * df + (lane & 15), 32 * c + 16 + 4 * g));
-            bf16x8 vfr;
-#pragma unroll
-            for (int e = 0; e < 4; ++e) {
-              vfr[e] = v0[e];
-              vfr[e + 4] = v1[e];
-            }
+            const bf16x8 vfr = tr_frag<D>(sV, c, df, lane);
 #pragma unroll
             for (int nf = 0; nf < 2; ++nf)
               acc_o[df][2 * hp + nf] = __builtin_amdgcn_mfma_f32_16x16x32_bf16(
@@ -277,7 +235,8 @@
 
 #pragma unroll
   for (int nf = 0; nf < NQ; ++nf) {
-    const int qg = wq0 + nf * 16 + (lane & 15);
+    const int qg = pair_row0<NQ>(q0, wave, nf >> 1) + (nf & 1) * 16 +
+                   (lane & 15);
     if (qg >= S) continue;
     const float lv = l_r[nf];
     const float inv = (lv > 0.f) ? 1.0f / lv : 0.f;
@@ -343,54 +302,9 @@
   }
 }
 
-template <int T, int D>
-DEV_INLINE void stage_nat_t(const bf16_t* __restrict__ src, int row0, int S,
-                            int64_t rs, bf16_t* nat, bf16_t* tr) {
-  constexpr int UN = T * D / 8 / NT;
-#pragma unroll
-  for (int u = 0; u < UN; ++u) {
-    const int idx = threadIdx.x + u * NT;
-    const int row = idx / (D / 8);
-    const int c = (idx % (D / 8)) * 8;
-    bf16x8 v8 = {};
-    if (row0 + row < S)
-      v8 = *reinterpret_cast<const bf16x8*>(
-          src + (int64_t)(row0 + row) * rs + c);
-    *reinterpret_cast<bf16x8*>(nat + loff<D>(row, c)) = v8;
-  }
-  constexpr int NSLAB = (T / 8) * (D / 2);
-#pragma unroll
-  for (int u = 0; u < (NSLAB + NT - 1) / NT; ++u) {
-    const int idx = threadIdx.x + u * NT;
-    if (idx < NSLAB) {
-      const int f = 2 * (idx % (D / 2));
-      const int kb = idx / (D / 2);
-      uint32_t r[8];
-#pragma unroll
-      for (int j = 0; j < 8; ++j) {
-        const int row = row0 + kb * 8 + j;
-        bf16x2 v2 = {};
-        if (row < S)
-          v2 = *reinterpret_cast<const bf16x2*>(src + (int64_t)row * rs + f);
-        r[j] = __builtin_bit_cast(uint32_t, v2);
-      }
-      uint32_t o0[4], o1[4];
-#pragma unroll
-      for (int d2 = 0; d2 < 4; ++d2) {
-        o0[d2] = __builtin_amdgcn_perm(r[2 * d2 + 1], r[2 * d2], 0x05040100u);
-        o1[d2] = __builtin_amdgcn_perm(r[2 * d2 + 1], r[2 * d2], 0x07060302u);
-      }
-      *reinterpret_cast<uint4*>(tr + loff<T>(f, kb * 8)) =
-          make_uint4(o0[0], o0[1], o0[2], o0[3]);
-      *reinterpret_cast<uint4*>(tr + loff<T>(f + 1, kb * 8)) =
-          make_uint4(o1[0], o1[1], o1[2], o1[3]);
-    }
-  }
-}
-
 constexpr int NTA = 512;
 
-template <int D, int PROBE = 0, int KBA = (D == 64 ? 256 : 128)>
+template <int D, int KBA = (D == 64 ? 256 : 128)>
 __launch_bounds__(NTA) __global__
 void flash_bwd_kv_kernel(const bf16_t* __restrict__ Q,
                          const bf16_t* __restrict__ K,
@@ -409,7 +323,7 @@
   const int bh = blockIdx.y;
   const int b = bh / H, h = bh % H;
   const int kv0 = blockIdx.x * KBA;
-  const int wave = threadIdx.x >> 6;
+  const int wave = __builtin_amdgcn_readfirstlane(threadIdx.x >> 6);
   const int lane = threadIdx.x & 63;
   const int g = lane >> 4;
 
@@ -420,14 +334,14 @@
   const bf16_t* vp = V + qoff;
   const bf16_t* dop = dO + ooff;
 
-  __shared__ bf16_t smem[KBA * D * 2 + QT * D * 2 + D * QT * 2];
+  __shared__ __attribute__((aligned(16))) bf16_t
+      smem[KBA * D * 2 + QT * D * 2];
   bf16_t* sKb = smem;
   bf16_t* sVb = sKb + KBA * D;
   bf16_t* sQ = sVb + KBA * D;
-  bf16_t* sQT = sQ + QT * D;
-  bf16_t* sdO = sQT + D * QT;
-  bf16_t* sdOT = sdO + QT * D;
-  __shared__ float sLSE[QT], sDELTA[QT];
+  bf16_t* sdO = sQ + QT * D;
+  __shared__ __attribute__((aligned(16))) float sNL2[QT], sDELTA[QT];
+  const float sl2 = scale * kLog2e;
 
   {
     constexpr int UN = KBA * D / 8 / NTA;
@@ -453,10 +367,7 @@
   f32x4 acc_dvT[NSL][DF] = {};
 
   constexpr int QUN = QT * D / 8 / NTA;
-  constexpr int TSLAB = (QT / 8) * (D / 2);
-  constexpr int TUN = (TSLAB + NTA - 1) / NTA;
   bf16x8 qn[QUN], don[QUN];
-  uint32_t qt[TUN][8], dot_[TUN][8];
   float lse2[QT / NTA + 1], dl2[QT / NTA + 1];
 
   auto tile_load = [&](int q0) {
@@ -475,29 +386,10 @@
       qn[u] = a;
       don[u] = b2;
     }
-#pragma unroll
-    for (int u = 0; u < TUN; ++u) {
-      const int idx = threadIdx.x + u * NTA;
-      if (idx >= TSLAB) break;
-      const int f = 2 * (idx % (D / 2));
-      const int kb = idx / (D / 2);
-#pragma unroll
-      for (int j = 0; j < 8; ++j) {
-        const int row = q0 + kb * 8 + j;
-        bf16x2 a = {}, b2 = {};
-        if (row < S) {
-          a = *reinterpret_cast<const bf16x2*>(
-              qp + (int64_t)row * q_rs + f);
-          b2 = *reinterpret_cast<const bf16x2*>(
-              dop + (int64_t)row * o_rs + f);
-        }
-        qt[u][j] = __builtin_bit_cast(uint32_t, a);
-        dot_[u][j] = __builtin_bit_cast(uint32_t, b2);
-      }
-    }
     for (int i = threadIdx.x, s2 = 0; i < QT; i += NTA, ++s2) {
       const int qg = q0 + i;
-      lse2[s2] = (qg < S) ? LSE[(int64_t)bh * S + qg] : -3.0e38f;
+      const float l = (qg < S) ? LSE[(int64_t)bh * S + qg] : -3.0e38f;
+      lse2[s2] = (l > -1.0e38f) ? -l * kLog2e : -3.0e38f;
       dl2[s2] = (qg < S) ? DELTA[(int64_t)bh * S + qg] : 0.f;
     }
   };
@@ -510,38 +402,8 @@
       *reinterpret_cast<bf16x8*>(sQ + loff<D>(row, c)) = qn[u];
       *reinterpret_cast<bf16x8*>(sdO + loff<D>(row, c)) = don[u];
     }
-#pragma unroll
-    for (int u = 0; u < TUN; ++u) {
-      const int idx = threadIdx.x + u * NTA;
-      if (idx >= TSLAB) break;
-      const int f = 2 * (idx % (D / 2));
-      const int kb = idx / (D / 2);
-      uint32_t o0[4], o1[4];
-#pragma unroll
-      for (int d2 = 0; d2 < 4; ++d2) {
-        o0[d2] = __builtin_amdgcn_perm(qt[u][2 * d2 + 1], qt[u][2 * d2],
-                                       0x05040100u);
-        o1[d2] = __builtin_amdgcn_perm(qt[u][2 * d2 + 1], qt[u][2 * d2],
-                                       0x07060302u);
-      }
-      *reinterpret_cast<uint4*>(sQT + loff<QT>(f, kb * 8)) =
-          make_uint4(o0[0], o0[1], o0[2], o0[3]);
-      *reinterpret_cast<uint4*>(sQT + loff<QT>(f + 1, kb * 8)) =
-          make_uint4(o1[0], o1[1], o1[2], o1[3]);
-#pragma unroll
-      for (int d2 = 0; d2 < 4; ++d2) {
-        o0[d2] = __builtin_amdgcn_perm(dot_[u][2 * d2 + 1], dot_[u][2 * d2],
-                                       0x05040100u);
-        o1[d2] = __builtin_amdgcn_perm(dot_[u][2 * d2 + 1], dot_[u][2 * d2],
-                                       0x07060302u);
-      }
-      *reinterpret_cast<uint4*>(sdOT + loff<QT>(f, kb * 8)) =
-          make_uint4(o0[0], o0[1], o0[2], o0[3]);
-      *reinterpret_cast<uint4*>(sdOT + loff<QT>(f + 1, kb * 8)) =
-          make_uint4(o1[0], o1[1], o1[2], o1[3]);
-    }
     for (int i = threadIdx.x, s2 = 0; i < QT; i += NTA, ++s2) {
-      sLSE[i] = lse2[s2];
+      sNL2[i] = lse2[s2];
       sDELTA[i] = dl2[s2];
     }
   };
@@ -555,6 +417,7 @@
 
 #pragma unroll
     for (int sl = 0; sl < NSL; ++sl) {
+      if (causal && kv0 + sl * 128 + wave * 16 > q0 + QT - 1) continue;
       f32x4 st[4] = {};
       f32x4 dpt[4] = {};
 #pragma unroll
@@ -583,19 +446,20 @@
       const bool winner = (!causal || kvb + wave * 16 + 15 < q0) &&
                           q0 + QT <= S && kvb + 128 <= S;
       if (winner) {
-        f32x4 lsev[4], dlv[4];
+        f32x4 nl2v[4], dlv[4];
 #pragma unroll
         for (int mi = 0; mi < 4; ++mi) {
-          lsev[mi] = *reinterpret_cast<const f32x4*>(sLSE + 16 * mi + 4 * g);
+          nl2v[mi] = *reinterpret_cast<const f32x4*>(sNL2 + 16 * mi + 4 * g);
           dlv[mi] = *reinterpret_cast<const f32x4*>(sDELTA + 16 * mi + 4 * g);
         }
 #pragma unroll
         for (int mi = 0; mi < 4; ++mi)
 #pragma unroll
           for (int e = 0; e < 4; ++e) {
-            const float pt = fast_exp(st[mi][e] * scale - lsev[mi][e]);
+            const float pt = __builtin_amdgcn_exp2f(
+                __builtin_fmaf(st[mi][e], sl2, nl2v[mi][e]));
             st[mi][e] = pt;
-            dpt[mi][e] = pt * (dpt[mi][e] - dlv[mi][e]) * scale;
+            dpt[mi][e] = pt * (dpt[mi][e] - dlv[mi][e]);
           }
       } else {
 #pragma unroll
@@ -604,14 +468,15 @@
           for (int e = 0; e < 4; ++e) {
             const int qrow = 16 * mi + 4 * g + e;
             const int qg = q0 + qrow;
-            const float lse = sLSE[qrow];
+            const float nl2 = sNL2[qrow];
             const float dl = sDELTA[qrow];
             const bool valid = qg < S && kvg < S && (!causal || kvg <= qg) &&
-                               lse > -1.0e38f;
-            const float arg = valid ? st[mi][e] * scale - lse : -3.0e38f;
-            const float pt = fast_exp(arg);
+                               nl2 > -1.0e38f;
+            const float arg =
+                valid ? __builtin_fmaf(st[mi][e], sl2, nl2) : -3.0e38f;
+            const float pt = __builtin_amdgcn_exp2f(arg);
             st[mi][e] = pt;
-            dpt[mi][e] = pt * (dpt[mi][e] - dl) * scale;
+            dpt[mi][e] = pt * (dpt[mi][e] - dl);
           }
       }
 
@@ -628,23 +493,8 @@
         }
 #pragma unroll
         for (int df = 0; df < DF; ++df) {
-          const int fr = PROBE ? 0 : (lane & 15);
-          const bf16x4 a0 = *reinterpret_cast<const bf16x4*>(
-              sdOT + loff<QT>(16 * df + fr, 32 * c + 4 * g));
-          const bf16x4 a1 = *reinterpret_cast<const bf16x4*>(
-              sdOT + loff<QT>(16 * df + fr, 32 * c + 16 + 4 * g));
-          const bf16x4 q0f = *reinterpret_cast<const bf16x4*>(
-              sQT + loff<QT>(16 * df + fr, 32 * c + 4 * g));
-          const bf16x4 q1f = *reinterpret_cast<const bf16x4*>(
-              sQT + loff<QT>(16 * df + fr, 32 * c + 16 + 4 * g));
-          bf16x8 afr, qfr;
-#pragma unroll
-          for (int e = 0; e < 4; ++e) {
-            afr[e] = a0[e];
-            afr[e + 4] = a1[e];
-            qfr[e] = q0f[e];
-            qfr[e + 4] = q1f[e];
-          }
+          const bf16x8 afr = tr_frag<D>(sdO, c, df, lane);
+          const bf16x8 qfr = tr_frag<D>(sQ, c, df, lane);
           acc_dvT[sl][df] = __builtin_amdgcn_mfma_f32_16x16x32_bf16(
               afr, pb, acc_dvT[sl][df], 0, 0, 0);
           acc_dkT[sl][df] = __builtin_amdgcn_mfma_f32_16x16x32_bf16(
@@ -669,7 +519,7 @@
         bf16x4 kv4, vv4;
 #pragma unroll
         for (int e = 0; e < 4; ++e) {
-          kv4[e] = f2bf(acc_dkT[sl][df][e]);
+          kv4[e] = f2bf(acc_dkT[sl][df][e] * scale);
           vv4[e] = f2bf(acc_dvT[sl][df][e]);
         }
         const int64_t off = qoff + (int64_t)kvg * q_rs + 16 * df + 4 * g;
@@ -700,10 +550,9 @@
   const int bh = blockIdx.y;
   const int b = bh / H, h = bh % H;
   const int q0 = blockIdx.x * (128 * NQ);
-  const int wave = threadIdx.x >> 6;
+  const int wave = __builtin_amdgcn_readfirstlane(threadIdx.x >> 6);
   const int lane = threadIdx.x & 63;
   const int g = lane >> 4;
-  const int wq0 = q0 + wave * 16 * NQ;
 
   const int64_t qoff = (int64_t)b * q_bs + (int64_t)h * q_hs;
   const int64_t ooff = (int64_t)b * o_bs + (int64_t)h * o_hs;
@@ -713,17 +562,19 @@
   const bf16_t* dop = dO + ooff;
   bf16_t* dqp = dQ + qoff;
 
-  __shared__ bf16_t smem[KB * D * 2 + D * KB];
+  __shared__ __attribute__((aligned(16))) bf16_t smem[KB * D * 2];
   bf16_t* sK = smem;
   bf16_t* sV = smem + KB * D;
-  bf16_t* sKT = sV + KB * D;
-
+
+  const float sl2 = scale * kLog2e;
   bf16x8 qf[NQ][DK], dof[NQ][DK];
-  float lse_r[NQ], dl_r[NQ];
+  float nl2_r[NQ], dl_r[NQ];
 #pragma unroll
   for (int nf = 0; nf < NQ; ++nf) {
-    const int row = wq0 + nf * 16 + (lane & 15);
-    lse_r[nf] = (row < S) ? LSE[(int64_t)bh * S + row] : -3.0e38f;
+    const int row = pair_row0<NQ>(q0, wave, nf >> 1) + (nf & 1) * 16 +
+                    (lane & 15);
+    const float l = (row < S) ? LSE[(int64_t)bh * S + row] : -3.0e38f;
+    nl2_r[nf] = (l > -1.0e38f) ? -l * kLog2e : -3.0e38f;
     dl_r[nf] = (row < S) ? DELTA[(int64_t)bh * S + row] : 0.f;
 #pragma unroll
     for (int kk = 0; kk < DK; ++kk) {
@@ -742,10 +593,7 @@
   f32x4 acc_dq[DF][NQ] = {};
 
   constexpr int KUN = KB * D / 8 / NTB;
-  constexpr int NSLAB = (KB / 8) * (D / 2);
-  constexpr int SUN = (NSLAB + NTB - 1) / NTB;
   bf16x8 krg[KUN], vrg[KUN];
-  uint32_t ktr[SUN][8];
 
   auto stage_load = [&](int kv0) {
 #pragma unroll
@@ -763,21 +611,6 @@
       krg[u] = kv8;
       vrg[u] = vv8;
     }
-#pragma unroll
-    for (int u = 0; u < SUN; ++u) {
-      const int idx = threadIdx.x + u * NTB;
-      if (idx >= NSLAB) break;
-      const int f = 2 * (idx % (D / 2));
-      const int kb = idx / (D / 2);
-#pragma unroll
-      for (int j = 0; j < 8; ++j) {
-        const int kv = kv0 + kb * 8 + j;
-        bf16x2 v2 = {};
-        if (kv < S)
-          v2 = *reinterpret_cast<const bf16x2*>(kp + (int64_t)kv * q_rs + f);
-        ktr[u][j] = __builtin_bit_cast(uint32_t, v2);
-      }
-    }
   };
   auto stage_write = [&]() {
 #pragma unroll
@@ -788,25 +621,6 @@
       *reinterpret_cast<bf16x8*>(sK + loff<D>(row, c)) = krg[u];
       *reinterpret_cast<bf16x8*>(sV + loff<D>(row, c)) = vrg[u];
     }
-#pragma unroll
-    for (int u = 0; u < SUN; ++u) {
-      const int idx = threadIdx.x + u * NTB;
-      if (idx >= NSLAB) break;
-      const int f = 2 * (idx % (D / 2));
-      const int kb = idx / (D / 2);
-      uint32_t o0[4], o1[4];
-#pragma unroll
-      for (int d2 = 0; d2 < 4; ++d2) {
-        o0[d2] = __builtin_amdgcn_perm(ktr[u][2 * d2 + 1], ktr[u][2 * d2],
-                                       0x05040100u);
-        o1[d2] = __builtin_amdgcn_perm(ktr[u][2 * d2 + 1], ktr[u][2 * d2],
-                                       0x07060302u);
-      }
-      *reinterpret_cast<uint4*>(sKT + loff<KB>(f, kb * 8)) =
-          make_uint4(o0[0], o0[1], o0[2], o0[3]);
-      *reinterpret_cast<uint4*>(sKT + loff<KB>(f + 1, kb * 8)) =
-          make_uint4(o1[0], o1[1], o1[2], o1[3]);
-    }
   };
 
   const int kv_end = causal ? min(S, q0 + 128 * NQ) : S;
@@ -816,10 +630,10 @@
   for (int kv0 = 0; kv0 < kv_end; kv0 += KB) {
     if (kv0 + KB < kv_end) stage_load(kv0 + KB);
 
-    if (!causal || kv0 <= wq0 + 16 * NQ - 1) {
+    if (!causal || kv0 <= pair_row0<NQ>(q0, wave, NQ / 2 - 1) + 31) {
 #pragma unroll
      for (int hp = 0; hp < NQ / 2; ++hp) {
-      const int pq0 = wq0 + 32 * hp;
+      const int pq0 = pair_row0<NQ>(q0, wave, hp);
       if (causal && kv0 > pq0 + 31) continue;
       const bool inner = kv0 + KB <= pq0 && kv0 + KB <= S && pq0 + 32 <= S;
       bf16x4 dsb[4][2];
@@ -850,9 +664,10 @@
           if (inner) {
 #pragma unroll
             for (int e = 0; e < 4; ++e) {
-              const float pt = fast_exp(st[nf][e] * scale - lse_r[nfg]);
+              const float pt = __builtin_amdgcn_exp2f(
+                  __builtin_fmaf(st[nf][e], sl2, nl2_r[nfg]));
               dsb[mi][nf][e] =
-                  f2bf(pt * (dpt[nf][e] - dl_r[nfg]) * scale);
+                  f2bf(pt * (dpt[nf][e] - dl_r[nfg]));
             }
           } else {
 #pragma unroll
@@ -860,12 +675,13 @@
               const int kg = kv0 + 16 * mi + 4 * g + e;
               const bool valid = qg < S && kg < S &&
                                  (!causal || kg <= qg) &&
-                                 lse_r[nfg] > -1.0e38f;
-              const float arg = valid ? st[nf][e] * scale - lse_r[nfg]
-                                      : -3.0e38f;
-              const float pt = fast_exp(arg);
+                                 nl2_r[nfg] > -1.0e38f;
+              const float arg =
+                  valid ? __builtin_fmaf(st[nf][e], sl2, nl2_r[nfg])
+                        : -3.0e38f;
+              const float pt = __builtin_amdgcn_exp2f(arg);
               dsb[mi][nf][e] =
-                  f2bf(pt * (dpt[nf][e] - dl_r[nfg]) * scale);
+                  f2bf(pt * (dpt[nf][e] - dl_r[nfg]));
             }
           }
         }
@@ -883,16 +699,7 @@
           }
 #pragma unroll
         for (int df = 0; df < DF; ++df) {
-          const bf16x4 k0 = *reinterpret_cast<const bf16x4*>(
-              sKT + loff<KB>(16 * df + (lane & 15), 32 * c + 4 * g));
-          const bf16x4 k1 = *reinterpret_cast<const bf16x4*>(
-              sKT + loff<KB>(16 * df + (lane & 15), 32 * c + 16 + 4 * g));
-          bf16x8 kfr;
-#pragma unroll
-          for (int e = 0; e < 4; ++e) {
-            kfr[e] = k0[e];
-            kfr[e + 4] = k1[e];
-          }
+          const bf16x8 kfr = tr_frag<D>(sK, c, df, lane);
 #pragma unroll
           for (int nf = 0; nf < 2; ++nf)
             acc_dq[df][2 * hp + nf] = __builtin_amdgcn_mfma_f32_16x16x32_bf16(
@@ -911,13 +718,14 @@
 
 #pragma unroll
   for (int nf = 0; nf < NQ; ++nf) {
-    const int qg = wq0 + nf * 16 + (lane & 15);
+    const int qg = pair_row0<NQ>(q0, wave, nf >> 1) + (nf & 1) * 16 +
+                   (lane & 15);
     if (qg >= S) continue;
 #pragma unroll
     for (int df = 0; df < DF; ++df) {
       bf16x4 v4;
 #pragma unroll
-      for (int e = 0; e < 4; ++e) v4[e] = f2bf(acc_dq[df][nf][e]);
+      for (int e = 0; e < 4; ++e) v4[e] = f2bf(acc_dq[df][nf][e] * scale);
       *reinterpret_cast<bf16x4*>(
           dqp + (int64_t)qg * q_rs + 16 * df + 4 * g) = v4;
     }
@@ -980,17 +788,6 @@
                        o_hs, o_rs);                                          \
     dim3 kgrid((S + (DD == 64 ? 255 : 127)) / (DD == 64 ? 256 : 128),       \
                B * H);                                                       \
-    static const bool kv_probe = std::getenv("TEPDIST_FLASH_PROBE");         \
-    if (kv_probe)                                                            \
-      hipLaunchKernelGGL((flash_bwd_kv_kernel<DD, 1>), kgrid, dim3(512), 0,  \
-                         stream, static_cast<const bf16_t*>(q),              \
-                         static_cast<const bf16_t*>(k),                      \
-                         static_cast<const bf16_t*>(v),                      \
-                         static_cast<const bf16_t*>(dout), lse, delta,       \
-                         static_cast<bf16_t*>(dk), static_cast<bf16_t*>(dv), \
-                         S, H, scale, causal, q_bs, q_hs, q_rs, o_bs, o_hs,  \
-                         o_rs);                                              \
-    else                                                                     \
     hipLaunchKernelGGL(flash_bwd_kv_kernel<DD>, kgrid, dim3(512), 0, stream, \
                        static_cast<const bf16_t*>(q),                        \
                        static_cast<const bf16_t*>(k),                        \
diff --git a/tepdist_amd/ops/csrc/bindings.cpp b/tepdist_amd/ops/csrc/bindings.cpp
--- a/tepdist_amd/ops/csrc/bindings.cpp
+++ b/tepdist_amd/ops/csrc/bindings.cpp
@@ -313,6 +313,10 @@
                S(stream));
   });
 
+  m.def("tr16_frag_probe", [](uintptr_t out, int C, uintptr_t stream) {
+    tr16_frag_probe(reinterpret_cast<int*>(out), C, S(stream));
+  });
+
   m.def("adamw_mt", [](uintptr_t tabs, uintptr_t numel, uintptr_t wds,
                        uintptr_t ptypes, uintptr_t chunks, int nchunks,
                        int nt, float lr, float b1, float b2, float eps,
diff --git a/tepdist_amd/ops/csrc/debug.hip b/tepdist_amd/ops/csrc/debug.hip
--- a/tepdist_amd/ops/csrc/debug.hip
+++ b/tepdist_amd/ops/csrc/debug.hip
@@ -1,6 +1,7 @@
 
 #include "common.h"
 #include "kernels.h"
+#include "lds_frag.h"
 
 namespace tepdist {
 
@@ -26,6 +27,41 @@
   }
 }
 
+template <int C>
+__global__ void tr16_frag_probe_kernel(int* out) {
+  __shared__ __attribute__((aligned(16))) bf16_t img[64 * C];
+  for (int i = threadIdx.x; i < 64 * C; i += 64) {
+    const int row = i / C, col = i % C;
+    reinterpret_cast<unsigned short*>(img)[loff<C>(row, col)] =
+        (unsigned short)(row * 128 + col);
+  }
+  __syncthreads();
+  const int lane = threadIdx.x;
+#pragma unroll
+  for (int c = 0; c < 2; ++c)
+#pragma unroll
+    for (int df = 0; df < C / 16; ++df) {
+      const s16x8 bits =
+          __builtin_bit_cast(s16x8, tr_frag<C>(img, c, df, lane));
+#pragma unroll
+      for (int e = 0; e < 8; ++e)
+        out[((c * (C / 16) + df) * 64 + lane) * 8 + e] =
+            (unsigned short)bits[e];
+    }
+}
+
+}
+
+void tr16_frag_probe(int* out, int C, hipStream_t stream) {
+  if (C == 64)
+    hipLaunchKernelGGL(tr16_frag_probe_kernel<64>, dim3(1), dim3(64), 0,
+                       stream, out);
+  else if (C == 128)
+    hipLaunchKernelGGL(tr16_frag_probe_kernel<128>, dim3(1), dim3(64), 0,
+                       stream, out);
+  else
+    throw std::runtime_error("tr16_frag_probe: C must be 64 or 128");
+  HIP_CHECK(hipGetLastError());
 }
 
 void tr16_probe(float* out_pattern, float* out_uniform, hipStream_t stream) {
diff --git a/tepdist_amd/ops/csrc/kernels.h b/tepdist_amd/ops/csrc/kernels.h
--- a/tepdist_amd/ops/csrc/kernels.h
+++ b/tepdist_amd/ops/csrc/kernels.h
@@ -110,6 +110,7 @@
                    float bc2, const float* hyper, hipStream_t stream);
 
 void tr16_probe(float* out_pattern, float* out_uniform, hipStream_t stream);
+void tr16_frag_probe(int* out, int C, hipStream_t stream);
 
 void rmsnorm_fwd_bf16(const void* x, const void* g, void* y, float* rstd,
                       int64_t rows, int cols, float eps, hipStream_t stream);
diff --git a/tepdist_amd/ops/csrc/lds_frag.h b/tepdist_amd/ops/csrc/lds_frag.h
--- /dev/null
+++ b/tepdist_amd/ops/csrc/lds_frag.h
@@ -0,0 +1,34 @@
+#pragma once
+
+#include "common.h"
+
+namespace tepdist {
+
+template <int C>
+DEV_INLINE int loff(int row, int col_e) {
+  const int r1 = row >> 1;
+  const int x = ((r1 & 1) << 2) | (r1 & 2) | ((r1 >> 2) & 1);
+  return row * C + (col_e ^ ((x << 3) & (C - 1)));
+}
+
+typedef __attribute__((address_space(3))) bf16x4* lds_bf16x4_ptr;
+
+template <int C>
+DEV_INLINE bf16x8 tr_frag(const bf16_t* img, int c, int df, int lane) {
+  const int i = lane & 15, g = lane >> 4;
+  const int row = 32 * c + 4 * g + (i >> 2);
+  const int col = 16 * df + 4 * (i & 3);
+  const bf16x4 lo = __builtin_amdgcn_ds_read_tr16_b64_v4bf16(
+      (lds_bf16x4_ptr)(img + loff<C>(row, col)));
+  const bf16x4 hi = __builtin_amdgcn_ds_read_tr16_b64_v4bf16(
+      (lds_bf16x4_ptr)(img + loff<C>(row + 16, col)));
+  bf16x8 f;
+#pragma unroll
+  for (int e = 0; e < 4; ++e) {
+    f[e] = lo[e];
+    f[e + 4] = hi[e];
+  }
+  return f;
+}
+
+}
```
